# astaka-pe/SeMIGCN

Hardware: AMD Instinct MI355X
Metric: GCN train iters/sec + edges-aggregated/sec, 1M-vert mesh (higher is better)
Workload: dtype bf16 storage / f32 accumulate; 1 GPU; SGCN train iteration (13 ChebConv K=3 + BN + LeakyReLU, fwd+loss+bwd, Adam every 5th) on a closed torus mesh 1000x1000: V=1000000 E=6000000 directed, grid vertex order, bf16 features; V=1000000, E=6000000, vertex_order=grid

## Files before the change

include/semigcn.h:

```cpp
#ifndef SEMIGCN_H
#define SEMIGCN_H

#include <stdint.h>

#ifdef __cplusplus
extern "C" {
#endif

#if defined(__GNUC__)
#define SG_API __attribute__((visibility("default")))
#else
#define SG_API
#endif

#define SG_ABI_VERSION 1

enum sg_status {
  SG_OK = 0,
  SG_ERR_INVALID = -1,
  SG_ERR_HIP = -2,
  SG_ERR_UNSUPPORTED = -3,
  SG_ERR_NO_DEVICE = -4
};

enum sg_dtype {
  SG_F32 = 0,
  SG_BF16 = 1
};

typedef struct sg_graph sg_graph;
typedef struct sg_pool sg_pool;

SG_API const char* sg_last_error(void);
SG_API int sg_abi_version(void);
SG_API int sg_device_count(void);

SG_API int sg_graph_create(const int64_t* edge_index, int64_t E, int64_t V, void* stream, sg_graph** out);

SG_API int sg_graph_create_rect(const int64_t* dst, const int64_t* src, int64_t n, int64_t V_dst,
                         int64_t V_src, const float* dis_src, void* stream, sg_graph** out);

SG_API int sg_graph_create_rows(const int64_t* dst_pos, const int64_t* src, int64_t n, int64_t n_rows, int64_t V_src,
                                const int32_t* row_id, const float* dis_rows, const float* dis_src, void* stream,
                                sg_graph** out);

SG_API int sg_graph_destroy(sg_graph* g);

typedef struct sg_graph_info {
  int64_t V_dst, V_src;
  int64_t nnz;
  int32_t symmetric;
  int32_t max_degree;
} sg_graph_info;
SG_API int sg_graph_query(const sg_graph* g, sg_graph_info* info);
SG_API int sg_graph_is_reordered(const sg_graph* g);
SG_API int sg_graph_export(const sg_graph* g, int32_t* rowptr, int32_t* colidx, float* dis, void* stream);

SG_API int sg_graph_prepare(const sg_graph* g, int64_t C, int dtype, void* stream);
SG_API int sg_spmm(const sg_graph* g, int transpose, const void* X, int64_t ldx, const void* X0,
            int64_t ldx0, const void* X1, int64_t ldx1, void* Y, int64_t ldy, int64_t C, int dtype,
            float alpha, float beta, float gamma, void* stream);

SG_API int sg_pool_create(const int64_t* fine, const int64_t* coarse, int64_t n, int64_t n_fine,
                   int64_t n_coarse, void* stream, sg_pool** out);
SG_API int sg_pool_destroy(sg_pool* p);
SG_API int sg_pool_mean(const sg_pool* p, const void* X, int64_t ldx, void* Y, int64_t ldy, int64_t C,
                 int dtype, void* stream);
SG_API int sg_pool_mean_bwd(const sg_pool* p, const void* dY, int64_t lddy, void* dX, int64_t lddx,
                     int64_t C, int dtype, void* stream);
SG_API int sg_unpool(const sg_pool* p, const void* X, int64_t ldx, void* Y, int64_t ldy, int64_t C,
              int dtype, void* stream);
SG_API int sg_unpool_bwd(const sg_pool* p, const void* dY, int64_t lddy, void* dX, int64_t lddx,
                  int64_t C, int dtype, void* stream);

SG_API int sg_gather_rows(const int32_t* rows, int64_t n, const void* X, int64_t ldx, void* Y,
                   int64_t ldy, int64_t C, int dtype, void* stream);

SG_API int sg_thin_supported(int64_t N, int64_t K);
SG_API int64_t sg_thin_tn_blocks(int64_t V);
SG_API int sg_thin_nt(const void* X, int64_t ldx, const float* W, int64_t ldw, const float* bias, void* Y, int64_t ldy,
                      int64_t V, int64_t N, int64_t K, int dtype, void* stream);
SG_API int sg_thin_tn(const void* A, int64_t lda, const void* B, int64_t ldb, int64_t V, int64_t N, int64_t K, int dtype,
                      float* workspace, float* out, int64_t ldo, void* stream);
SG_API int64_t sg_col_apply_blocks(int64_t V, int64_t C, int dtype);
SG_API int sg_bn_act_bwd_apply_colsum(const void* dA, int64_t ldda, const void* H, int64_t ldh, const float* scale,
                                      const float* shift, const float* mean, const float* invstd, const float* k,
                                      const float* c1, const float* c2, float slope, void* dH, int64_t lddh, int64_t V,
                                      int64_t C, int dtype, float* colsum_partial, float* colsum, void* stream);
SG_API int64_t sg_col_blocks(int64_t V);
SG_API int sg_col_moments(const void* X, int64_t ldx, int64_t V, int64_t C, int dtype, float* partial,
                          int64_t nb, void* stream);
SG_API int sg_bn_merge(const float* partial, int64_t nb, int64_t V, int64_t C, float* stats, void* stream);
SG_API int sg_bn_stats_finalize(const float* partial, int64_t nb, int64_t V, int64_t C, const float* gamma,
                                const float* beta, float* running_mean, float* running_var, float momentum, float eps,
                                float* out, int64_t* batches_tracked, void* stream);
SG_API int sg_bn_bwd_coeffs(const float* partial, int64_t nb, int64_t C, double N, const float* gamma,
                            const float* invstd, float* out, float* acc_dweight, float* acc_dbias, const float* count_dev,
                            void* stream);
SG_API int sg_bn_merge_tiles(const float* partial, int64_t n_tiles, int64_t rows_per_tile, int64_t V, int64_t C, float* stats,
                             float* count_out, void* stream);
SG_API int sg_bn_finalize_ranks(const float* all, int64_t world, int64_t C, const float* gamma, const float* beta,
                                float* running_mean, float* running_var, float momentum, float eps, float* out,
                                float* out_n, int64_t* batches_tracked, void* stream);
SG_API int sg_multi_add(int64_t n, const float* const* srcs, const int64_t* src_ld, const int64_t* rows, const int64_t* cols,
                        float* const* dsts, void* stream);
SG_API int sg_bn_finalize(const float* stats, double N, int64_t C, const float* gamma, const float* beta,
                          float* running_mean, float* running_var, float momentum, float eps, float* out,
                          void* stream);
SG_API int sg_scale_shift_act(const void* X, int64_t ldx, const float* scale, const float* shift, float slope,
                              void* Y, int64_t ldy, int64_t V, int64_t C, int dtype, void* stream);
SG_API int sg_bn_act_bwd_reduce(const void* dA, int64_t ldda, const void* H, int64_t ldh, const float* scale,
                                const float* shift, const float* mean, const float* invstd, float slope,
                                float* partial, int64_t nb, int64_t V, int64_t C, int dtype, void* stream);
SG_API int sg_bn_act_bwd_apply(const void* dA, int64_t ldda, const void* H, int64_t ldh, const float* scale,
// ... 209 lines not shown
```

semigcn_amd/capi.py:

```python
from __future__ import annotations

import ctypes
import functools
from array import array as _array
import os
from ctypes import POINTER, byref, c_char_p, c_float, c_int, c_int32, c_int64, c_void_p
from typing import Optional

import torch

_LIB_NAME = "libsemigcn_hip.so"
_LIB_PATH = os.path.join(os.path.dirname(os.path.abspath(__file__)), _LIB_NAME)

SG_F32, SG_BF16 = 0, 1
_DTYPES = {torch.float32: SG_F32, torch.bfloat16: SG_BF16}


class SemigcnLibraryError(RuntimeError):
    """libsemigcn_hip.so is absent / unloadable, or a call into it failed."""


class sg_graph_info(ctypes.Structure):
    _fields_ = [("V_dst", c_int64), ("V_src", c_int64), ("nnz", c_int64),
                ("symmetric", c_int32), ("max_degree", c_int32)]
# ... 1 lines not shown

class sg_block(ctypes.Structure):
    _fields_ = [("graph", c_void_p), ("pool", c_void_p),
                ("pool_mode", c_int32), ("dtype", c_int32), ("K", c_int32), ("order", c_int32), ("training", c_int32),
                ("refresh_weights", c_int32), ("need_dx", c_int32), ("reserved_", c_int32),
                ("V", c_int64), ("V_out", c_int64), ("Cin", c_int64), ("Cout", c_int64),
                ("momentum", c_float), ("eps", c_float), ("slope", c_float), ("reserved2_", c_float),
                ("W", c_void_p * 3), ("bias", c_void_p), ("gamma", c_void_p), ("beta", c_void_p),
                ("running_mean", c_void_p), ("running_var", c_void_p), ("batches_tracked", c_void_p),
                ("wpack", c_void_p), ("wpack_t", c_void_p), ("wpack32", c_void_p), ("wpack32_t", c_void_p), ("bias_k", c_void_p),
                ("wsplit", c_void_p), ("wsplit_t", c_void_p),
                ("X", c_void_p), ("ldx", c_int64), ("T", c_void_p), ("ldt", c_int64), ("H", c_void_p), ("stats", c_void_p),
                ("Y", c_void_p), ("ldy", c_int64),
                ("dY", c_void_p), ("lddy", c_int64), ("dX", c_void_p), ("lddx", c_int64), ("dW", c_void_p), ("dvec", c_void_p),
                ("acc_W", c_void_p * 3), ("acc_bias", c_void_p), ("acc_gamma", c_void_p), ("acc_beta", c_void_p),
                ("ws", c_void_p), ("ws_bytes", c_int64),
                ("phase", c_int32), ("world", c_int32), ("graph_wide", c_void_p), ("V_ext", c_int64), ("ldh", c_int64),
                ("local", c_void_p), ("stats_rows", c_void_p), ("gathered", c_void_p), ("gathered_ready", c_int32),
                ("reserved3_", c_int32), ("count", c_void_p), ("send_index", c_void_p), ("n_send", c_int64), ("send", c_void_p),
                ("recv", c_void_p), ("G", c_void_p)]


PHASE_CONV, PHASE_BN, PHASE_BWD_REDUCE, PHASE_BWD_A, PHASE_BWD_B = 1, 2, 4, 8, 16


class sg_part_step(ctypes.Structure):
    _fields_ = [("kind", c_int32), ("reserved_", c_int32), ("blocks", POINTER(sg_block)), ("n", c_int64),
                ("send", c_void_p), ("recv", c_void_p)]


STEP_BLOCKS, STEP_EXCHANGE, STEP_ALL_REDUCE, STEP_ALL_GATHER = 0, 1, 2, 3


class sg_trace_record(ctypes.Structure):
    _fields_ = [("kind", c_int32), ("dtype", c_int32), ("engine", c_int32), ("reserved_", c_int32),
                ("a", c_int64), ("b", c_int64), ("c", c_int64), ("ms", c_float), ("reserved2_", c_float)]


_SIGNATURES = {
    "sg_last_error": (c_char_p, []),
    "sg_abi_version": (c_int, []),
    "sg_device_count": (c_int, []),
    "sg_graph_create": (c_int, [c_void_p, c_int64, c_int64, c_void_p, POINTER(c_void_p)]),
    "sg_graph_create_rect": (c_int, [c_void_p, c_void_p, c_int64, c_int64, c_int64, c_void_p, c_void_p,
                                     POINTER(c_void_p)]),
    "sg_graph_create_rows": (c_int, [c_void_p, c_void_p, c_int64, c_int64, c_int64, c_void_p, c_void_p, c_void_p, c_void_p,
                                     POINTER(c_void_p)]),
    "sg_graph_destroy": (c_int, [c_void_p]),
    "sg_graph_query": (c_int, [c_void_p, POINTER(sg_graph_info)]),
    "sg_graph_is_reordered": (c_int, [c_void_p]),
    "sg_graph_export": (c_int, [c_void_p, c_void_p, c_void_p, c_void_p, c_void_p]),
    "sg_spmm": (c_int, [c_void_p, c_int, c_void_p, c_int64, c_void_p, c_int64, c_void_p, c_int64,
                        c_void_p, c_int64, c_int64, c_int, c_float, c_float, c_float, c_void_p]),
    "sg_graph_prepare": (c_int, [c_void_p, c_int64, c_int, c_void_p]),
    "sg_pool_create": (c_int, [c_void_p, c_void_p, c_int64, c_int64, c_int64, c_void_p, POINTER(c_void_p)]),
    "sg_pool_destroy": (c_int, [c_void_p]),
    "sg_pool_mean": (c_int, [c_void_p, c_void_p, c_int64, c_void_p, c_int64, c_int64, c_int, c_void_p]),
    "sg_pool_mean_bwd": (c_int, [c_void_p, c_void_p, c_int64, c_void_p, c_int64, c_int64, c_int, c_void_p]),
    "sg_unpool": (c_int, [c_void_p, c_void_p, c_int64, c_void_p, c_int64, c_int64, c_int, c_void_p]),
    "sg_unpool_bwd": (c_int, [c_void_p, c_void_p, c_int64, c_void_p, c_int64, c_int64, c_int, c_void_p]),
    "sg_tuning_set": (c_int, [c_int, c_int]),
    "sg_mesh_loss_blocks": (c_int64, [c_int64, c_int64]),
    "sg_mesh_loss_fwd": (c_int, [c_void_p] * 6 + [c_int64, c_int64, c_void_p, c_void_p]),
    "sg_mesh_loss_bwd": (c_int, [c_void_p] * 7 + [c_int64, c_int64, c_int64, c_void_p, c_void_p]),
    "sg_mesh_loss_bwd_det": (c_int, [c_void_p] * 7 + [c_int64, c_int64, c_int64, c_void_p, c_void_p, c_void_p, c_void_p]),
    "sg_col_blocks": (c_int64, [c_int64]),
    "sg_col_moments": (c_int, [c_void_p, c_int64, c_int64, c_int64, c_int, c_void_p, c_int64, c_void_p]),
    "sg_bn_merge": (c_int, [c_void_p, c_int64, c_int64, c_int64, c_void_p, c_void_p]),
    "sg_bn_stats_finalize": (c_int, [c_void_p, c_int64, c_int64, c_int64, c_void_p, c_void_p, c_void_p, c_void_p, c_float,
                                     c_float, c_void_p, c_void_p, c_void_p]),
    "sg_bn_stats_finalize_tiles": (c_int, [c_void_p, c_int64, c_int64, c_int64, c_int64, c_void_p, c_void_p, c_void_p,
                                           c_void_p, c_float, c_float, c_void_p, c_void_p, c_void_p]),
    "sg_gemm_nt_takes_big_tile": (c_int, [c_int64, c_int64, c_int64, c_int64, c_int64, c_int64]),
    "sg_gemm_tile_rows": (c_int64, [c_int64]),
    "sg_gemm_row_tiles": (c_int64, [c_int64, c_int64]),
    "sg_gemm_nt": (c_int, [c_void_p, c_int64, c_void_p, c_int64, c_void_p, c_void_p, c_int64, c_int64, c_int64, c_int64,
                           c_int, c_void_p, c_void_p]),
    "sg_gemm_nt_f32_supported": (c_int, [c_int64, c_int64, c_int64, c_int64, c_int64]),
    "sg_gemm_nt_f32_pays": (c_int, [c_int64, c_int64, c_int64]),
    "sg_gemm_nt_f32_variant": (c_int, [c_int64]),
    "sg_gemm_nt_f32_workspace": (c_int64, [c_int64, c_int64]),
    "sg_gemm_nt_f32": (c_int, [c_void_p, c_int64, c_void_p, c_int64, c_int64, c_void_p, c_void_p, c_int64, c_int64, c_int64,
                               c_int64, c_void_p, c_int64, c_void_p]),
    "sg_gemm_tn_f32_supported": (c_int, [c_int64, c_int64, c_int64, c_int64, c_int64]),
    "sg_gemm_tn_f32_workspace": (c_int64, [c_int64, c_int64, c_int64]),
    "sg_gemm_tn_f32": (c_int, [c_void_p, c_int64, c_void_p, c_int64, c_int64, c_int64, c_int64, c_void_p, c_int64, c_void_p,
                               c_int64, c_void_p]),
    "sg_gemm_tn_slabs": (c_int64, [c_int64, c_int64, c_int64]),
    "sg_gemm_tn_takes_big_tile": (c_int, [c_int64, c_int64, c_int64, c_int64, c_int64]),
    "sg_gemm_tn": (c_int, [c_void_p, c_int64, c_void_p, c_int64, c_int64, c_int64, c_int64, c_int, c_void_p, c_void_p, c_int64,
                           c_void_p]),
    "sg_thin_supported": (c_int, [c_int64, c_int64]),
    "sg_thin_tn_blocks": (c_int64, [c_int64]),
    "sg_thin_nt": (c_int, [c_void_p, c_int64, c_void_p, c_int64, c_void_p, c_void_p, c_int64, c_int64, c_int64, c_int64, c_int,
                           c_void_p]),
    "sg_thin_tn": (c_int, [c_void_p, c_int64, c_void_p, c_int64, c_int64, c_int64, c_int64, c_int, c_void_p, c_void_p, c_int64,
                           c_void_p]),
    "sg_bn_bwd_coeffs": (c_int, [c_void_p, c_int64, c_int64, ctypes.c_double, c_void_p, c_void_p, c_void_p, c_void_p,
                                 c_void_p, c_void_p, c_void_p]),
    "sg_bn_merge_tiles": (c_int, [c_void_p, c_int64, c_int64, c_int64, c_int64, c_void_p, c_void_p, c_void_p]),
    "sg_multi_add": (c_int, [c_int64, c_void_p, c_void_p, c_void_p, c_void_p, c_void_p, c_void_p]),
    "sg_input_bounds": (c_int, [c_void_p, c_int64, c_void_p, c_void_p, c_void_p, c_void_p, c_void_p]),
    "sg_input_prep_bwd_routed": (c_int, [c_void_p, c_int64, c_void_p, c_void_p, c_void_p, c_void_p, c_void_p, c_void_p, c_void_p,
                                         c_void_p, c_int64, c_int, c_void_p]),
    "sg_mesh_loss_finalize": (c_int, [c_void_p, c_int64, c_float, c_float, c_float, c_float, c_void_p, c_void_p]),
    "sg_bnf_blocks": (c_int64, [c_int64]),
# ... 203 lines not shown
        with _on_device(ei.device):
            _check(load().sg_graph_create(_ptr(ei), ei.shape[1], int(num_vertices), _stream(ei), byref(out)),
                   "sg_graph_create")
        return cls(out.value, ei.device)

    @classmethod
    def from_partition(cls, dst: torch.Tensor, src: torch.Tensor, n_owned: int, n_ext: int,
                       dis_ext: torch.Tensor) -> "GraphHandle":
        for t, n in ((dst, "dst"), (src, "src"), (dis_ext, "dis_ext")):
            _require_device(t, n)
        dst, src = dst.contiguous(), src.contiguous()
        dis_ext = dis_ext.contiguous().float()
        assert dst.dtype == torch.int64 and src.dtype == torch.int64 and dis_ext.numel() == n_ext
        out = c_void_p()
        with _on_device(dst.device):
            _check(load().sg_graph_create_rect(_ptr(dst), _ptr(src), dst.numel(), int(n_owned), int(n_ext),
                                               _ptr(dis_ext), _stream(dst), byref(out)),
                   "sg_graph_create_rect")
        return cls(out.value, dst.device)

    @classmethod
    def from_rows(cls, dst_pos: torch.Tensor, src: torch.Tensor, row_id: torch.Tensor, out_rows: int, n_ext: int,
                  dis_rows: torch.Tensor, dis_ext: torch.Tensor) -> "GraphHandle":
        for t, n in ((dst_pos, "dst_pos"), (src, "src"), (row_id, "row_id"), (dis_rows, "dis_rows"), (dis_ext, "dis_ext")):
            _require_device(t, n)
        dst_pos, src = dst_pos.contiguous().long(), src.contiguous().long()
        row_id = row_id.contiguous().to(torch.int32)
        dis_rows, dis_ext = dis_rows.contiguous().float(), dis_ext.contiguous().float()
        assert dis_rows.numel() == row_id.numel() and dis_ext.numel() == n_ext
        out = c_void_p()
        with _on_device(src.device):
            _check(load().sg_graph_create_rows(_ptr(dst_pos), _ptr(src), dst_pos.numel(), row_id.numel(), int(n_ext),
                                               _ptr(row_id), _ptr(dis_rows), _ptr(dis_ext), _stream(src), byref(out)),
                   "sg_graph_create_rows")
        h = cls(out.value, src.device)
        h.num_rows = int(out_rows)
        return h

    def arrays(self):
        rp = torch.empty(self.num_rows + 1, dtype=torch.int32, device=self.device)
        ci = torch.empty(self.nnz, dtype=torch.int32, device=self.device)
        ds = torch.empty(self.num_cols, dtype=torch.float32, device=self.device)
        with _on_device(self.device):
            _check(load().sg_graph_export(self._h, _ptr(rp), _ptr(ci), _ptr(ds), _stream(rp)), "sg_graph_export")
        return rp, ci, ds

    def prepare(self, C: int, dtype: torch.dtype) -> None:
        with _on_device(self.device):
            _check(load().sg_graph_prepare(self._h, int(C), _DTYPES[dtype], torch.cuda.current_stream(self.device).cuda_stream),
                   "sg_graph_prepare")

    def spmm(self, X: torch.Tensor, Y: torch.Tensor, *, alpha: float = 1.0, X0: Optional[torch.Tensor] = None,
             beta: float = 0.0, X1: Optional[torch.Tensor] = None, gamma: float = 0.0,
             transpose: bool = False) -> torch.Tensor:
        if _timer is None and X.is_cuda and X.dim() == 2 and Y.dim() == 2 and X.device.index == _current_device():
            dt = X.dtype
            code = _DTYPES.get(dt)
            C = X.shape[1]
            n_in, n_out = (self.num_rows, self.num_cols) if transpose else (self.num_cols, self.num_rows)
            sx, sy = X.stride(), Y.stride()
            ok = (code is not None and X.shape[0] == n_in and Y.dtype == dt and Y.device == X.device and Y.shape[0] == n_out
                  and Y.shape[1] == C and (C <= 1 or (sx[1] == 1 and sy[1] == 1)))
            p0 = l0 = p1 = l1 = 0
            if ok and X0 is not None:
                s0 = X0.stride()
                ok = (X0.dtype == dt and X0.device == X.device and X0.dim() == 2 and X0.shape[0] == n_out and X0.shape[1] == C
                      and (C <= 1 or s0[1] == 1))
                p0, l0 = X0.data_ptr(), (s0[0] if n_out > 1 else max(s0[0], C))
            if ok and X1 is not None:
                s1 = X1.stride()
                ok = (X1.dtype == dt and X1.device == X.device and X1.dim() == 2 and X1.shape[0] == n_out and X1.shape[1] == C
                      and (C <= 1 or s1[1] == 1))
                p1, l1 = X1.data_ptr(), (s1[0] if n_out > 1 else max(s1[0], C))
            if ok and _raw_stream is not None:
                rc = _lib.sg_spmm(self._h, 1 if transpose else 0, X.data_ptr(), sx[0] if n_in > 1 else max(sx[0], C),
                                  p0, l0, p1, l1, Y.data_ptr(), sy[0] if n_out > 1 else max(sy[0], C), C, code,
                                  alpha, beta, gamma, _raw_stream(X.device.index))
                if rc:
                    _check(rc, "sg_spmm")
                return Y
        return self._spmm_checked(X, Y, alpha, X0, beta, X1, gamma, transpose)

    def _spmm_checked(self, X, Y, alpha, X0, beta, X1, gamma, transpose) -> torch.Tensor:
        for t, n in ((X, "X"), (Y, "Y"), (X0, "X0"), (X1, "X1")):
            if t is not None:
                _require_device(t, n)
                if t.dtype != X.dtype:
                    raise SemigcnLibraryError(f"{n} dtype {t.dtype} != X dtype {X.dtype}")
        C = X.shape[1]
        n_in, n_out = (self.num_rows, self.num_cols) if transpose else (self.num_cols, self.num_rows)
        if X.shape[0] != n_in or Y.shape != (n_out, C):
            raise SemigcnLibraryError(f"spmm shape mismatch: X {tuple(X.shape)} Y {tuple(Y.shape)} "
                                      f"operator {n_out}x{n_in}")
        for t, n in ((X0, "X0"), (X1, "X1")):
            if t is not None and t.shape != (n_out, C):
                raise SemigcnLibraryError(f"{n} shape {tuple(t.shape)} != {(n_out, C)}")
        timer = _timer
        with _on_device(X.device):
            if timer is not None:
                ev0, ev1 = torch.cuda.Event(enable_timing=True), torch.cuda.Event(enable_timing=True)
                ev0.record()
            _check(load().sg_spmm(self._h, int(transpose), _ptr(X), _rows2d(X, "X"),
                                  _ptr(X0), 0 if X0 is None else _rows2d(X0, "X0"),
                                  _ptr(X1), 0 if X1 is None else _rows2d(X1, "X1"),
                                  _ptr(Y), _rows2d(Y, "Y"), C, dtype_code(X),
                                  float(alpha), float(beta), float(gamma), _stream(X)), "sg_spmm")
            if timer is not None:
                ev1.record()
                n_epi = int(X0 is not None) + int(X1 is not None)
                timer.records.append(((C, str(X.dtype).replace("torch.", ""), n_epi, self.rows_processed), ev0, ev1))
        return Y

    def dilate_bits(self, bits: torch.Tensor) -> torch.Tensor:
        _require_device(bits, "bits")
        if bits.dtype != torch.int64 or bits.dim() != 2 or bits.shape[0] != self.num_rows:
            raise SemigcnLibraryError(f"bits must be int64 [{self.num_rows}, W], got {bits.dtype} {tuple(bits.shape)}")
        bits = bits.contiguous()
        out = torch.empty_like(bits)
        with _on_device(bits.device):
            _check(load().sg_mask_dilate(self._h, _ptr(bits), _ptr(out), bits.shape[1], _stream(bits)),
                   "sg_mask_dilate")
        return out

    def close(self):
        if getattr(self, "_h", None) is not None and self._h.value:
            load().sg_graph_destroy(self._h)
            self._h = c_void_p(0)

    def __del__(self):
        try:
            self.close()
        except Exception:
            pass

# ... 127 lines not shown
    rpt = int(rows_per_tile) if rows_per_tile else (int(num_rows) + nb - 1) // nb
    base = out.data_ptr()
    with _on_device(partial.device):
        _check(load().sg_bn_merge_tiles(_ptr(partial), nb, rpt, int(num_rows), C, base, base + 8 * C, _stream(partial)),
               "sg_bn_merge_tiles")
    return out


def bn_finalize(stats: torch.Tensor, count: float, gamma: torch.Tensor, beta: torch.Tensor,
                running_mean: Optional[torch.Tensor], running_var: Optional[torch.Tensor], momentum: float,
                eps: float) -> torch.Tensor:
    C = stats.shape[1]
    out = torch.empty((4, C), dtype=torch.float32, device=stats.device)
    for t, n in ((running_mean, "running_mean"), (running_var, "running_var")):
        if t is not None:
            _f32vec(t, C, n)
    with _on_device(stats.device):
        _check(load().sg_bn_finalize(_ptr(stats), float(count), C, _ptr(_f32vec(gamma, C, "weight")),
                                     _ptr(_f32vec(beta, C, "bias")), _ptr(running_mean), _ptr(running_var),
                                     float(momentum), float(eps), _ptr(out), _stream(stats)), "sg_bn_finalize")
    return out


def bn_finalize_ranks(all_stats: torch.Tensor, gamma: torch.Tensor, beta: torch.Tensor,
                      running_mean: Optional[torch.Tensor], running_var: Optional[torch.Tensor], momentum: float,
                      eps: float, batches_tracked: Optional[torch.Tensor] = None):
    world, w = all_stats.shape
    C = (w - 1) // 2
    out = torch.empty((4, C), dtype=torch.float32, device=all_stats.device)
    n = torch.empty((1,), dtype=torch.float32, device=all_stats.device)
    with _on_device(all_stats.device):
        _check(load().sg_bn_finalize_ranks(_ptr(all_stats), world, C, _ptr(_f32vec(gamma, C, "weight")),
                                           _ptr(_f32vec(beta, C, "bias")), _ptr(running_mean), _ptr(running_var),
                                           float(momentum), float(eps), _ptr(out), _ptr(n),
                                           _counter(batches_tracked, all_stats), _stream(all_stats)),
               "sg_bn_finalize_ranks")
    return out, n


def bn_stats_finalize(partial: torch.Tensor, num_rows: int, gamma: torch.Tensor, beta: torch.Tensor,
                      running_mean: Optional[torch.Tensor], running_var: Optional[torch.Tensor], momentum: float,
                      eps: float, batches_tracked: Optional[torch.Tensor] = None) -> torch.Tensor:
    nb, _, C = partial.shape
    out = torch.empty((4, C), dtype=torch.float32, device=partial.device)
    for t, n in ((running_mean, "running_mean"), (running_var, "running_var")):
        if t is not None:
            _f32vec(t, C, n)
    with _on_device(partial.device):
        _check(load().sg_bn_stats_finalize(_ptr(partial), nb, int(num_rows), C, _ptr(_f32vec(gamma, C, "weight")),
                                           _ptr(_f32vec(beta, C, "bias")), _ptr(running_mean), _ptr(running_var),
                                           float(momentum), float(eps), _ptr(out), _counter(batches_tracked, partial),
                                           _stream(partial)), "sg_bn_stats_finalize")
    return out


def bn_stats_finalize_tiles(partial: torch.Tensor, rows_per_tile: int, num_rows: int, gamma: torch.Tensor,
                            beta: torch.Tensor, running_mean: Optional[torch.Tensor], running_var: Optional[torch.Tensor],
                            momentum: float, eps: float, batches_tracked: Optional[torch.Tensor] = None) -> torch.Tensor:
    nb, _, C = partial.shape
    out = torch.empty((4, C), dtype=torch.float32, device=partial.device)
    for t, n in ((running_mean, "running_mean"), (running_var, "running_var")):
        if t is not None:
            _f32vec(t, C, n)
    with _on_device(partial.device):
        _check(load().sg_bn_stats_finalize_tiles(_ptr(partial), nb, int(rows_per_tile), int(num_rows), C,
                                                 _ptr(_f32vec(gamma, C, "weight")), _ptr(_f32vec(beta, C, "bias")),
                                                 _ptr(running_mean), _ptr(running_var), float(momentum), float(eps),
                                                 _ptr(out), _counter(batches_tracked, partial), _stream(partial)),
               "sg_bn_stats_finalize_tiles")
    return out


def gemm_tile_rows(N: int) -> int:
    return _sizes("sg_gemm_tile_rows", int(N))


def gemm_nt_supported(A: torch.Tensor, B: torch.Tensor, ldc: int) -> bool:
    if A.dtype != torch.bfloat16 or B.dtype != torch.bfloat16 or not A.is_cuda or A.dim() != 2 or B.dim() != 2:
        return False
    if A.shape[1] != B.shape[1] or A.stride(1) != 1 or B.stride(1) != 1 or A.shape[0] == 0:
        return False
    K, N = A.shape[1], B.shape[0]
    return (K % 8 == 0 and N % 8 == 0 and A.stride(0) % 8 == 0 and B.stride(0) % 8 == 0 and ldc % 8 == 0
            and A.data_ptr() % 16 == 0 and B.data_ptr() % 16 == 0)


def gemm_nt_takes_big_tile(M: int, N: int, K: int, lda: int, ldb: int, ldc: int) -> bool:
    return bool(_sizes("sg_gemm_nt_takes_big_tile", int(M), int(N), int(K), int(lda), int(ldb), int(ldc)))


def gemm_nt(A: torch.Tensor, B: torch.Tensor, bias: Optional[torch.Tensor] = None, out: Optional[torch.Tensor] = None,
            moments: bool = False):
    _require_device(A, "A")
    _require_device(B, "B")
    M, K = A.shape
    N = B.shape[0]
    if out is None:
        out = torch.empty((M, N), dtype=torch.bfloat16, device=A.device)
    if out.shape != (M, N) or out.dtype != torch.bfloat16 or B.shape[1] != K:
        raise SemigcnLibraryError(f"gemm_nt shape mismatch: A {tuple(A.shape)} B {tuple(B.shape)} out {tuple(out.shape)}")
    if bias is not None:
        _f32vec(bias, N, "bias")
    mom = None
    if moments:
        mom = torch.empty((_sizes("sg_gemm_row_tiles", M, N), 2, N), dtype=torch.float32, device=A.device)
    with _on_device(A.device):
# ... 707 lines not shown
```

semigcn_amd/csrc/api.hip:

```cpp
#include <stdarg.h>

#include <new>

#include <mutex>

#include "sg_common.h"

namespace sg {

static thread_local std::string t_error;

void set_error(const char* fmt, ...) {
  char buf[1024];
  va_list ap;
  va_start(ap, fmt);
  vsnprintf(buf, sizeof(buf), fmt, ap);
  va_end(ap);
  t_error = buf;
}

namespace {

struct ScopedFree {
  void* p = nullptr;
  ~ScopedFree() { if (p) (void)hipFree(p); }
};

void destroy_graph(sg_graph* g) {
  if (!g) return;
  g->fwd.release();
  g->bwd.release();
  g->loc.release();
  if (g->row_id) (void)hipFree(g->row_id);
  if (g->dis_dst_loc) (void)hipFree(g->dis_dst_loc);
  if (g->dis_src && g->dis_src != g->dis_dst) (void)hipFree(g->dis_src);
  if (g->dis_dst) (void)hipFree(g->dis_dst);
  delete g;
}

void destroy_pool(sg_pool* p) {
  if (!p) return;
  p->by_coarse.release();
  p->by_fine.release();
  if (p->inv_count) (void)hipFree(p->inv_count);
  delete p;
}

int check_dense(const char* what, const void* X, int64_t ld, int64_t C) {
  SG_REQUIRE(X != nullptr, "%s: null pointer", what);
  SG_REQUIRE(ld >= C, "%s: row stride %lld < C %lld", what, (long long)ld, (long long)C);
  return SG_OK;
}

std::mutex g_rec_mu;
int build_pending_records(const Csr& c_, hipStream_t stream) {
  hipStreamCaptureStatus st = hipStreamCaptureStatusNone;
  if (hipStreamIsCapturing(stream, &st) != hipSuccess) (void)hipGetLastError();
  if (st != hipStreamCaptureStatusNone) return SG_OK;
  std::lock_guard<std::mutex> lock(g_rec_mu);
  Csr& c = const_cast<Csr&>(c_);
  if (!__atomic_load_n(&c.rec_pending, __ATOMIC_ACQUIRE)) return SG_OK;
  const int rc = build_ring_records(&c, c.pend_scale_src, c.pend_scale_dst, c.pend_row_id, stream);
  if (rc == SG_OK) __atomic_store_n(&c.rec_pending, false, __ATOMIC_RELEASE);
  return rc;
}

int run_csr(const Csr& c, const float* sd, const float* ss, const void* X, int64_t ldx,
            const void* X0, int64_t ldx0, const void* X1, int64_t ldx1, void* Y, int64_t ldy,
            int64_t C, int dtype, float alpha, float beta, float gamma, hipStream_t stream,
            const int32_t* row_id = nullptr) {
  SG_REQUIRE(C >= 0 && C <= INT32_MAX, "C out of range");
  if (c.n_rows == 0 || C == 0) return SG_OK;
  int rc;
  if ((rc = check_dense("X", X, ldx, C)) != SG_OK) return rc;
  if ((rc = check_dense("Y", Y, ldy, C)) != SG_OK) return rc;
  if (X0 && (rc = check_dense("X0", X0, ldx0, C)) != SG_OK) return rc;
  if (X1 && (rc = check_dense("X1", X1, ldx1, C)) != SG_OK) return rc;
  SG_REQUIRE(X != Y, "Y must not alias X");
  if (__atomic_load_n(&c.rec_pending, __ATOMIC_ACQUIRE) && (dtype == SG_BF16 || (dtype == SG_F32 && ring_f32_enabled())) && (C == 128 || C == 256) &&
      (rc = build_pending_records(c, stream)) != SG_OK)
    return rc;
  SpmmArgs a;
  a.rowptr = c.rowptr;
  a.idx = c.idx;
  if (c.tile_rows == kTileRows) {
    a.tile_uptr = c.tile_uptr;
    a.tile_uniq = c.tile_uniq;
    a.tile_eloc = c.tile_eloc;
  }
  if (ss != nullptr && ss == c.packed_scale) {
    a.idx_w = c.idx_w;
    a.tile_uniq_w = c.tile_uniq_w;
    if (c.lt_uptr && c.lt_uniq_w && c.idx_w) {
      a.lt_idx_w = c.idx_w;
      a.lt_uptr = c.lt_uptr;
      a.lt_eloc = c.lt_eloc;
      a.lt_uniq_w = c.lt_uniq_w;
    }
  }
  if (ss != nullptr && ss == c.packed_scale && c.lt_rec && sd == c.rec_scale_dst && row_id == c.rec_row_id) {
    a.lt_rec = c.lt_rec;
    a.lt_nrec = c.lt_nrec;
    a.lt_idx_w = c.idx_w;
  }
  a.row_id = row_id;
  a.scale_dst = sd;
  a.scale_src = ss;
  a.X = X; a.X0 = X0; a.X1 = X1; a.Y = Y;
  a.ldx = ldx; a.ldx0 = X0 ? ldx0 : 0; a.ldx1 = X1 ? ldx1 : 0; a.ldy = ldy;
  a.n_rows = (int32_t)c.n_rows;
  a.n_cols = c.n_cols;
  a.C = (int32_t)C;
  a.alpha = alpha; a.beta = beta; a.gamma = gamma;
  return launch_spmm(a, dtype, stream);
}

}
}

using namespace sg;

extern "C" {

SG_API const char* sg_last_error(void) { return t_error.c_str(); }

SG_API int sg_abi_version(void) { return SG_ABI_VERSION; }

SG_API int sg_device_count(void) {
  int n = 0;
  hipError_t e = hipGetDeviceCount(&n);
  if (e != hipSuccess) {
    set_error("hipGetDeviceCount failed: %s", hipGetErrorString(e));
    (void)hipGetLastError();
    return SG_ERR_NO_DEVICE;
  }
  return n;
}

SG_API int sg_graph_create(const int64_t* edge_index, int64_t E, int64_t V, void* stream_, sg_graph** out) {
  SG_REQUIRE(out != nullptr, "sg_graph_create: out is null");
  *out = nullptr;
  SG_REQUIRE(E >= 0 && V >= 0, "sg_graph_create: negative size");
  SG_REQUIRE(E == 0 || edge_index != nullptr, "sg_graph_create: edge_index is null");
  hipStream_t stream = (hipStream_t)stream_;
  sg_graph* g = new (std::nothrow) sg_graph();
  SG_REQUIRE(g != nullptr, "out of host memory");
  const int64_t* src = edge_index;
  const int64_t* dst = edge_index + E;
  ScopedFree kf, kb;
  int rc = SG_OK;
  do {
    if (E > 0) {
      if (hipMalloc(&kf.p, E * sizeof(uint64_t)) != hipSuccess ||
          hipMalloc(&kb.p, E * sizeof(uint64_t)) != hipSuccess) {
        set_error("hipMalloc of sort keys failed");
        rc = SG_ERR_HIP;
        break;
      }
    }
    if ((rc = build_csr(dst, src, E, V, V, true, stream, &g->fwd, (uint64_t*)kf.p)) != SG_OK) break;
    if ((rc = build_csr(src, dst, E, V, V, true, stream, &g->bwd, (uint64_t*)kb.p)) != SG_OK) break;
    if (hipMalloc((void**)&g->dis_dst, (V > 0 ? V : 1) * sizeof(float)) != hipSuccess) {
      set_error("hipMalloc of dis failed");
      rc = SG_ERR_HIP;
      break;
    }
    g->dis_src = g->dis_dst;
// ... 113 lines not shown
    if (rc == SG_OK) rc = pack_source_scale(&g->fwd, g->dis_src, stream);
    if (rc == SG_OK && ring_enabled()) g->fwd.defer_records(g->dis_src, g->dis_dst, g->row_id);
    if (rc == SG_OK && hipStreamSynchronize(stream) != hipSuccess) {
      set_error("stream sync failed in sg_graph_create_rows");
      rc = SG_ERR_HIP;
    }
  }
  if (rc != SG_OK) {
    destroy_graph(g);
    return rc;
  }
  g->symmetric = true;
  g->square = false;
  *out = g;
  return SG_OK;
}

SG_API int sg_graph_destroy(sg_graph* g) {
  destroy_graph(g);
  return SG_OK;
}

SG_API int sg_graph_query(const sg_graph* g, sg_graph_info* info) {
  SG_REQUIRE(g && info, "sg_graph_query: null argument");
  info->V_dst = g->fwd.n_rows;
  info->V_src = g->fwd.n_cols;
  info->nnz = g->fwd.nnz;
  info->symmetric = g->symmetric ? 1 : 0;
  info->max_degree = g->fwd.max_degree;
  return SG_OK;
}

SG_API int sg_graph_is_reordered(const sg_graph* g) {
  if (!g) {
    set_error("sg_graph_is_reordered: null graph");
    return SG_ERR_INVALID;
  }
  return (g->square && g->row_id) ? 1 : 0;
}

SG_API int sg_graph_export(const sg_graph* g, int32_t* rowptr, int32_t* colidx, float* dis, void* stream_) {
  SG_REQUIRE(g != nullptr, "sg_graph_export: null graph");
  hipStream_t stream = (hipStream_t)stream_;
  if (rowptr)
    SG_HIP_TRY(hipMemcpyAsync(rowptr, g->fwd.rowptr, (g->fwd.n_rows + 1) * sizeof(int32_t),
                              hipMemcpyDeviceToDevice, stream));
  if (colidx && g->fwd.nnz > 0)
    SG_HIP_TRY(hipMemcpyAsync(colidx, g->fwd.idx, g->fwd.nnz * sizeof(int32_t), hipMemcpyDeviceToDevice, stream));
  if (dis && g->fwd.n_cols > 0)
    SG_HIP_TRY(hipMemcpyAsync(dis, g->dis_src, g->fwd.n_cols * sizeof(float), hipMemcpyDeviceToDevice, stream));
  return SG_OK;
}

SG_API int sg_spmm(const sg_graph* g, int transpose, const void* X, int64_t ldx, const void* X0, int64_t ldx0,
            const void* X1, int64_t ldx1, void* Y, int64_t ldy, int64_t C, int dtype, float alpha,
            float beta, float gamma, void* stream) {
  SG_REQUIRE(g != nullptr, "sg_spmm: null graph");
  const bool t = transpose != 0;
  if (t && !g->square) {
    set_error("sg_spmm: transpose of a rectangular (partition) operator is not available; "
              "apply it owner-computes on exchanged gradient rows");
    return SG_ERR_UNSUPPORTED;
  }
  TraceScope trace(0, dtype, 0, C, (X0 ? 1 : 0) + (X1 ? 1 : 0), (t && !g->symmetric) ? g->bwd.n_rows : g->fwd.n_rows,
                   (hipStream_t)stream);
  if (g->square && g->symmetric && g->row_id && g->loc.rowptr)
    return run_csr(g->loc, g->dis_dst_loc, g->dis_src, X, ldx, X0, ldx0, X1, ldx1, Y, ldy, C, dtype, -alpha, beta, gamma,
                   (hipStream_t)stream, g->row_id);
  if (!g->square && g->row_id)
    return run_csr(g->fwd, g->dis_dst, g->dis_src, X, ldx, X0, ldx0, X1, ldx1, Y, ldy, C, dtype, -alpha, beta, gamma,
                   (hipStream_t)stream, g->row_id);
  const Csr& c = (t && !g->symmetric) ? g->bwd : g->fwd;
  return run_csr(c, g->dis_dst, g->dis_src, X, ldx, X0, ldx0, X1, ldx1, Y, ldy, C, dtype, -alpha,
                 beta, gamma, (hipStream_t)stream);
}

SG_API int sg_graph_prepare(const sg_graph* g, int64_t C, int dtype, void* stream) {
  SG_REQUIRE(g != nullptr, "sg_graph_prepare: null graph");
  if (!(C == 128 || C == 256) || !(dtype == SG_BF16 || (dtype == SG_F32 && ring_f32_enabled()))) return SG_OK;
  const Csr* all[3] = {&g->fwd, &g->bwd, &g->loc};
  for (const Csr* c : all) {
    if (!__atomic_load_n(&const_cast<Csr*>(c)->rec_pending, __ATOMIC_ACQUIRE)) continue;
    const int rc = build_pending_records(*c, (hipStream_t)stream);
    if (rc != SG_OK) return rc;
  }
  return SG_OK;
}

SG_API int sg_pool_create(const int64_t* fine, const int64_t* coarse, int64_t n, int64_t n_fine,
                   int64_t n_coarse, void* stream_, sg_pool** out) {
  SG_REQUIRE(out != nullptr, "sg_pool_create: out is null");
  *out = nullptr;
  SG_REQUIRE(n >= 0 && n_fine >= 0 && n_coarse >= 0, "sg_pool_create: negative size");
  hipStream_t stream = (hipStream_t)stream_;
  sg_pool* p = new (std::nothrow) sg_pool();
  SG_REQUIRE(p != nullptr, "out of host memory");
  int rc = build_csr(coarse, fine, n, n_coarse, n_fine, false, stream, &p->by_coarse, nullptr);
  if (rc == SG_OK) rc = build_csr(fine, coarse, n, n_fine, n_coarse, false, stream, &p->by_fine, nullptr);
  if (rc == SG_OK && hipMalloc((void**)&p->inv_count, (n_coarse > 0 ? n_coarse : 1) * sizeof(float)) != hipSuccess) {
    set_error("hipMalloc of inv_count failed");
    rc = SG_ERR_HIP;
  }
  if (rc == SG_OK) rc = degree_scale(p->by_coarse, false, p->inv_count, stream);
  if (rc == SG_OK && hipStreamSynchronize(stream) != hipSuccess) {
    set_error("stream sync failed in sg_pool_create");
    rc = SG_ERR_HIP;
  }
  if (rc != SG_OK) {
    destroy_pool(p);
    return rc;
  }
  *out = p;
  return SG_OK;
}

SG_API int sg_pool_destroy(sg_pool* p) {
  destroy_pool(p);
  return SG_OK;
}

SG_API int sg_pool_mean(const sg_pool* p, const void* X, int64_t ldx, void* Y, int64_t ldy, int64_t C, int dtype,
                 void* stream) {
  SG_REQUIRE(p != nullptr, "sg_pool_mean: null pool");
  TraceScope trace(3, dtype, 0, C, p->by_coarse.n_rows, p->by_coarse.n_cols, (hipStream_t)stream);
  return run_csr(p->by_coarse, p->inv_count, nullptr, X, ldx, nullptr, 0, nullptr, 0, Y, ldy, C, dtype,
                 1.f, 0.f, 0.f, (hipStream_t)stream);
}
// ... 109 lines not shown
                                const float* target_fn, const float* f_keep, const float* g, int64_t V, int64_t V_ext,
                                int64_t F, const sg_pool* incidence, float* corner_scratch, float* grad_pos, void* stream_) {
  SG_REQUIRE(V >= 0 && F >= 0 && V_ext >= V && g && (V_ext == 0 || grad_pos), "sg_mesh_loss_bwd_det: bad argument");
  SG_REQUIRE((V == 0 || (pos && target_pos && v_keep)) && (F == 0 || (pos && faces && target_fn && f_keep)),
             "sg_mesh_loss_bwd_det: null pointer");
  SG_REQUIRE(incidence && incidence->by_coarse.n_rows == V_ext && incidence->by_coarse.n_cols == 3 * F &&
                 (F == 0 || corner_scratch),
             "sg_mesh_loss_bwd_det: incidence must map the 3F face corners onto V_ext vertices");
  hipStream_t stream = (hipStream_t)stream_;
  int rc = launch_mesh_loss_bwd_corners(pos, faces, target_fn, f_keep, g, F, corner_scratch, stream);
  if (rc != SG_OK) return rc;
  if (V_ext == 0) return SG_OK;
  if (F == 0) {
    SG_HIP_TRY(hipMemsetAsync(grad_pos, 0, (size_t)V_ext * 3 * sizeof(float), stream));
  } else {
    rc = run_csr(incidence->by_coarse, nullptr, nullptr, corner_scratch, 3, nullptr, 0, nullptr, 0, grad_pos, 3, 3, SG_F32,
                 1.f, 0.f, 0.f, stream);
    if (rc != SG_OK) return rc;
  }
  return launch_mesh_loss_bwd_vertex_add(pos, target_pos, v_keep, g, V, grad_pos, stream);
}

SG_API int64_t sg_col_blocks(int64_t V) { return col_blocks(V); }

SG_API int sg_col_moments(const void* X, int64_t ldx, int64_t V, int64_t C, int dtype, float* partial, int64_t nb,
                          void* stream) {
  SG_REQUIRE(V >= 0 && C >= 0, "sg_col_moments: negative size");
  if (V == 0 || C == 0) return SG_OK;
  SG_REQUIRE(X && partial && ldx >= C, "sg_col_moments: bad argument");
  return launch_col_reduce(0, X, ldx, nullptr, 0, nullptr, nullptr, nullptr, nullptr, 0.f, partial, nb, V, C, dtype,
                           (hipStream_t)stream);
}

SG_API int sg_bn_merge(const float* partial, int64_t nb, int64_t V, int64_t C, float* stats, void* stream) {
  SG_REQUIRE(V > 0 && C >= 0 && partial && stats, "sg_bn_merge: bad argument");
  return launch_bn_merge(partial, nb, V, C, stats, (hipStream_t)stream);
}

SG_API int sg_bn_merge_tiles(const float* partial, int64_t n_tiles, int64_t rows_per_tile, int64_t V, int64_t C, float* stats,
                             float* count_out, void* stream) {
  SG_REQUIRE(V > 0 && C >= 0 && partial && stats, "sg_bn_merge_tiles: bad argument");
  return launch_bn_merge_tiles(partial, n_tiles, rows_per_tile, V, C, stats, count_out, (hipStream_t)stream);
}

SG_API int sg_bn_stats_finalize(const float* partial, int64_t nb, int64_t V, int64_t C, const float* gamma,
                                const float* beta, float* running_mean, float* running_var, float momentum, float eps,
                                float* out, int64_t* batches_tracked, void* stream) {
  SG_REQUIRE(V > 1 && C >= 0 && partial && gamma && beta && out, "sg_bn_stats_finalize: bad argument");
  SG_REQUIRE((running_mean == nullptr) == (running_var == nullptr),
             "sg_bn_stats_finalize: give both running buffers or none");
  return launch_bn_stats_finalize(partial, nb, V, C, gamma, beta, running_mean, running_var, momentum, eps, out,
                                  batches_tracked, (hipStream_t)stream);
}

SG_API int sg_bn_stats_finalize_tiles(const float* partial, int64_t n_tiles, int64_t rows_per_tile, int64_t V, int64_t C,
                                      const float* gamma, const float* beta, float* running_mean, float* running_var,
                                      float momentum, float eps, float* out, int64_t* batches_tracked, void* stream) {
  SG_REQUIRE(V > 1 && C >= 0 && partial && gamma && beta && out, "sg_bn_stats_finalize_tiles: bad argument");
  SG_REQUIRE((running_mean == nullptr) == (running_var == nullptr),
             "sg_bn_stats_finalize_tiles: give both running buffers or none");
  return launch_bn_stats_finalize_tiles(partial, n_tiles, rows_per_tile, V, C, gamma, beta, running_mean, running_var,
                                        momentum, eps, out, batches_tracked, (hipStream_t)stream);
}

SG_API int sg_gemm_nt_takes_big_tile(int64_t M, int64_t N, int64_t K, int64_t lda, int64_t ldb, int64_t ldc) {
  return gemm_nt_takes_big_tile(M, N, K, lda, ldb, ldc) ? 1 : 0;
}

SG_API int64_t sg_gemm_tile_rows(int64_t N) { return gemm_tile_rows(N); }

SG_API int64_t sg_gemm_row_tiles(int64_t M, int64_t N) {
  const int64_t r = gemm_tile_rows(N);
  return M <= 0 ? 0 : (M + r - 1) / r;
}

SG_API int sg_gemm_nt(const void* A, int64_t lda, const void* B, int64_t ldb, const float* bias, void* C, int64_t ldc,
                      int64_t M, int64_t N, int64_t K, int dtype, float* moments, void* stream) {
  SG_REQUIRE(M >= 0 && N >= 0 && K >= 0, "sg_gemm_nt: negative size");
  if (M == 0 || N == 0) return SG_OK;
  SG_REQUIRE(A && B && C && K > 0, "sg_gemm_nt: null operand or K = 0");
  SG_REQUIRE(lda >= K && ldb >= K && ldc >= N, "sg_gemm_nt: row stride shorter than the row");
  return launch_gemm_nt(A, lda, B, ldb, bias, C, ldc, M, N, K, dtype, moments, (hipStream_t)stream);
}

SG_API int64_t sg_gemm_tn_slabs(int64_t M, int64_t N, int64_t Kp) { return gemm_tn_slabs(M, N, Kp); }

SG_API int sg_gemm_tn_takes_big_tile(int64_t M, int64_t N, int64_t Kp, int64_t lda, int64_t ldb) {
  return gemm_tn_takes_big_tile(M, N, Kp, lda, ldb) ? 1 : 0;
}

SG_API int sg_gemm_tn(const void* A, int64_t lda, const void* B, int64_t ldb, int64_t M, int64_t N, int64_t Kp, int dtype,
                      float* workspace, float* out, int64_t ldo, void* stream) {
  SG_REQUIRE(M >= 0 && N >= 0 && Kp >= 0, "sg_gemm_tn: negative size");
  if (N == 0 || Kp == 0) return SG_OK;
  SG_REQUIRE(out != nullptr && ldo >= Kp, "sg_gemm_tn: bad output");
  if (M == 0) {
    SG_HIP_TRY(hipMemset2DAsync(out, ldo * sizeof(float), 0, Kp * sizeof(float), N, (hipStream_t)stream));
    return SG_OK;
  }
  SG_REQUIRE(A && B && workspace && lda >= N && ldb >= Kp, "sg_gemm_tn: null operand or short row stride");
  return launch_gemm_tn(A, lda, B, ldb, M, N, Kp, dtype, workspace, out, ldo, (hipStream_t)stream);
}

SG_API int sg_gemm_nt_f32_supported(int64_t M, int64_t N, int64_t K, int64_t lda, int64_t ldc) {
  return (gemm_nt_f32s_supported(M, N, K, lda, ldc) || (M >= 0 && mid_shape(N, K) && lda % 4 == 0 && ldc % 4 == 0)) ? 1 : 0;
}
// ... 253 lines not shown
```

semigcn_amd/csrc/block.hip:

```cpp
#include <math.h>

#include "sg_common.h"

namespace sg {
namespace {

bool g_block_planes = true;

inline int64_t esize(int dtype) { return dtype == SG_F32 ? 4 : 2; }
inline int64_t align_up(int64_t v) { return (v + 255) & ~(int64_t)255; }

struct Carver {
  char* base;
  int64_t cap, at = 0;
  bool overflow = false;
  Carver(void* b, int64_t c) : base((char*)b), cap(c) {}
  void* take(int64_t bytes) {
    const int64_t off = at;
    at += align_up(bytes > 0 ? bytes : 1);
    if (!base) return nullptr;
    if (at > cap) {
      overflow = true;
      return nullptr;
    }
// ... 88 lines not shown
  } else if (b.pool_mode == 2) {
    SG_REQUIRE(b.pool && b.pool->by_fine.n_cols == b.V && b.pool->by_fine.n_rows == b.V_out,
               "sg_block: MeshUnpool handle does not map %lld coarse rows onto %lld fine rows", (long long)b.V, (long long)b.V_out);
  } else {
    set_error("sg_block: pool_mode %d", b.pool_mode);
    return SG_ERR_INVALID;
  }
  if (b.training) SG_REQUIRE(b.V_out > 1, "sg_block: BatchNorm in training mode needs more than one row");
  s->V = b.V; s->Vo = b.V_out; s->Ci = b.Cin; s->Co = b.Cout; s->K = b.K;
  s->KCi = b.K * b.Cin; s->KCo = b.K * b.Cout; s->e = esize(b.dtype);
  if (col_apply_blocks(b.V_out, b.Cout, b.dtype) == 0) {
    set_error("sg_block: Cout = %lld is not served (whole 16-byte vectors, at most 256 of them per row)", (long long)b.Cout);
    return SG_ERR_UNSUPPORTED;
  }
  if (b.order == 0) {
    s->thin = thin_shape(s->Co, s->KCi);
    s->blas_fwd = !s->thin && !dense_nt_own(b.dtype, s->V, s->Co, s->KCi, s->KCi, s->KCi, s->Co);
    s->blas_dx = !s->thin && !dense_nt_own(b.dtype, s->V, s->KCi, s->Co, s->Co, s->Co, s->KCi);
    s->blas_dw = !s->thin && !dense_tn_own(b.dtype, s->V, s->Co, s->KCi, s->Co, s->KCi);
    s->tn_floats = dense_tn_workspace(b.dtype, s->V, s->Co, s->KCi);
  } else {
    s->thin = false;
    s->blas_fwd = !dense_nt_own(b.dtype, s->V, s->KCo, s->Ci, s->Ci, s->Ci, s->KCo);
    s->blas_dx = !dense_nt_own(b.dtype, s->V, s->Ci, s->KCo, s->KCo, s->KCo, s->Ci);
    s->blas_dw = !dense_tn_own(b.dtype, s->V, s->KCo, s->Ci, s->KCo, s->Ci) || thin_shape(s->KCo, s->Ci);
    s->tn_floats = thin_shape(s->KCo, s->Ci) ? 0 : dense_tn_workspace(b.dtype, s->V, s->KCo, s->Ci);
    if (thin_shape(s->KCo, s->Ci)) {
      set_error("sg_block: order 1 with a %lld x %lld weight stack is not served", (long long)s->KCo, (long long)s->Ci);
      return SG_ERR_UNSUPPORTED;
    }
  }
  {
    const int64_t C = b.order == 0 ? s->Ci : s->Co;
    int lg = 0;
    while ((1 << lg) < C) ++lg;
    bool ok = b.dtype == SG_BF16 && b.K > 1 && (1 << lg) == C && C >= 8 && C <= 64 && g_block_planes;
    if (ok && b.order == 0)
      ok = dense_planes_ok_nt(b.dtype, s->V, s->Co, s->KCi) && dense_planes_ok_nt(b.dtype, s->V, s->KCi, s->Co) &&
           dense_planes_ok_tn(b.dtype, s->V, s->Co, s->KCi);
    else if (ok)
      ok = dense_planes_ok_nt(b.dtype, s->V, s->KCo, s->Ci) && dense_planes_ok_nt(b.dtype, s->V, s->Ci, s->KCo) &&
           dense_planes_ok_tn(b.dtype, s->V, s->KCo, s->Ci);
    s->planes_ok = ok;
    s->pl = Planes{};
    if (ok) {
      s->pl.log2 = lg;
      s->pl.stride = s->V * C;
    }
  }
  s->nb = col_blocks(s->Vo);
  const int64_t R = gemm_tile_rows(s->Co);
  const int64_t tiles = (s->V + R - 1) / R;
  s->mom_floats = (tiles > s->nb ? tiles : s->nb) * 2 * s->Co;
  return SG_OK;
}

struct FwdWs {
  float* moments;
  void* Z;
  void* Hc;
  void* blas;
};
void carve_fwd(const sg_block& b, const Shape& s, Carver& c, FwdWs* w) {
  w->moments = (float*)c.take(s.mom_floats * 4);
  w->Z = b.order == 1 ? c.take(s.V * s.KCo * s.e) : nullptr;
  w->Hc = b.pool_mode ? c.take(s.V * s.Co * s.e) : nullptr;
  w->blas = s.blas_fwd ? c.take((int64_t)kBlasWorkspace) : nullptr;
}

struct BwdWs {
  float* part;
  float* colsum;
  void* dHp;
  void* dHc;
  void* G;
  float* tn;
  void* blas;
};
void carve_bwd(const sg_block& b, const Shape& s, Carver& c, BwdWs* w) {
  w->part = (float*)c.take(s.nb * 2 * s.Co * 4);
  w->colsum = (float*)c.take(col_apply_blocks(s.Vo, s.Co, b.dtype) * s.Co * 4);
  const bool sep = b.order == 0 || b.pool_mode != 0;
  w->dHp = sep ? c.take(s.Vo * s.Co * s.e) : nullptr;
  w->dHc = (b.order == 0 && b.pool_mode) ? c.take(s.V * s.Co * s.e) : nullptr;
  w->G = c.take(s.V * (b.order == 0 ? s.KCi : s.KCo) * s.e);
  w->tn = (float*)c.take(s.tn_floats * 4);
  w->blas = (s.blas_dx || s.blas_dw) ? c.take((int64_t)kBlasWorkspace) : nullptr;
}

int spmm(const sg_block& b, bool transpose, const void* X, int64_t ldx, const void* X0, int64_t ldx0, const void* X1,
         int64_t ldx1, void* Y, int64_t ldy, int64_t C, float alpha, float beta, float gamma, hipStream_t s) {
  return sg_spmm(b.graph, transpose ? 1 : 0, X, ldx, X0, ldx0, X1, ldx1, Y, ldy, C, b.dtype, alpha, beta, gamma, (void*)s);
}

inline char* col(void* base, int64_t cols, int64_t e) { return (char*)base + cols * e; }

inline bool split_image_shape(int64_t N, int64_t K) { return N >= 64 && N % 4 == 0 && K >= 64 && K % 32 == 0; }
inline const void* split_image(const sg_block& b, bool transposed, int64_t N, int64_t K) {
  return (b.dtype == SG_F32 && split_image_shape(N, K)) ? (transposed ? b.wsplit_t : b.wsplit) : nullptr;
}

int pack(const sg_block& b, hipStream_t stream) {
  SG_REQUIRE(b.wpack != nullptr, "sg_block: wpack is null");
  PackArgs a;
  for (int k = 0; k < 3; ++k) a.W[k] = k < b.K ? b.W[k] : nullptr;
  for (int k = 0; k < b.K; ++k) SG_REQUIRE(b.W[k] != nullptr, "sg_block: W[%d] is null", k);
  a.bias = b.bias;
  a.wpack = b.wpack; a.wpack_t = b.wpack_t; a.wpack32 = b.wpack32; a.wpack32_t = b.wpack32_t;
  a.bias_k = (b.order == 1 && b.bias) ? b.bias_k : nullptr;
  a.K = b.K; a.Cin = (int)b.Cin; a.Cout = (int)b.Cout; a.order = b.order; a.dtype = b.dtype;
  const int64_t n = (int64_t)b.K * b.Cin * b.Cout;
  pack_weights<<<(int)((n + 255) / 256), 256, 0, stream>>>(a);
  SG_HIP_TRY(hipGetLastError());
  if (b.dtype == SG_F32 && (b.wsplit || b.wsplit_t)) {
    const int64_t na = b.order == 0 ? b.Cout : (int64_t)b.K * b.Cout, ka = b.order == 0 ? (int64_t)b.K * b.Cin : b.Cin;
    const float* const w32 = (const float*)b.wpack;
    if (b.wsplit && split_image_shape(na, ka)) {
      int rc = launch_pack_split(w32, ka, 1, b.V, na, ka, b.wsplit, stream);
      if (rc != SG_OK) return rc;
    }
    if (b.wsplit_t && split_image_shape(ka, na)) {
      int rc = launch_pack_split(w32, 1, ka, b.V, ka, na, b.wsplit_t, stream);
      if (rc != SG_OK) return rc;
    }
  }
  return SG_OK;
}

int t_layout(const sg_block& b, const Shape& s, const char* who, Planes* pt) {
  *pt = Planes{};
  SG_REQUIRE(b.T != nullptr, "%s: order 0 needs the [V, K*Cin] buffer T", who);
  if (b.K > 1 && b.ldt == s.Ci) {
    SG_REQUIRE(s.planes_ok, "%s: T given as K planes (ldt == Cin) for a shape that does not take them (sg_block_planar)", who);
    *pt = s.pl;
    return SG_OK;
  }
  SG_REQUIRE(b.ldt >= s.KCi, "%s: row stride of T shorter than K*Cin", who);
  return SG_OK;
}

int forward(const sg_block& b, hipStream_t stream) {
  Shape s;
  int rc = shape_of(b, &s);
  if (rc != SG_OK) return rc;
  SG_REQUIRE(b.X && b.H && b.Y && b.stats && b.gamma && b.beta && b.wpack, "sg_block_forward: null pointer");
  SG_REQUIRE(b.ldy >= s.Co && b.ldx >= s.Ci, "sg_block_forward: row stride shorter than the row");
  SG_REQUIRE((b.running_mean == nullptr) == (b.running_var == nullptr), "sg_block_forward: give both running buffers or none");
  SG_REQUIRE(b.training || b.running_mean, "sg_block_forward: eval mode needs the running statistics");
  if (s.thin) SG_REQUIRE(b.wpack32 && b.wpack32_t, "sg_block_forward: a tiny weight matrix needs wpack32 / wpack32_t");
  if (b.order == 1 && b.bias) SG_REQUIRE(b.bias_k != nullptr, "sg_block_forward: order 1 with a bias needs bias_k");
  Carver c(b.ws, b.ws_bytes);
  FwdWs w;
  carve_fwd(b, s, c, &w);
  SG_REQUIRE(b.ws != nullptr && !c.overflow, "sg_block_forward: scratch too small (%lld bytes given, %lld needed)",
             (long long)b.ws_bytes, (long long)c.at);
  if (b.refresh_weights && (rc = pack(b, stream)) != SG_OK) return rc;

  void* const Hc = b.pool_mode ? w.Hc : b.H;
  bool tile_moments = false;
  if (b.order == 0) {
    Planes pt;
    if ((rc = t_layout(b, s, "sg_block_forward", &pt)) != SG_OK) return rc;
    auto t = [&](int k) { return pt.on() ? col(b.T, k * pt.stride, s.e) : col(b.T, k * s.Ci, s.e); };
    if (b.X != b.T && (rc = copy_rows(b.X, b.ldx, b.T, b.ldt, s.V, s.Ci, b.dtype, stream)) != SG_OK) return rc;
    for (int k = 1; k < b.K; ++k) {
      rc = spmm(b, false, t(k - 1), b.ldt, k >= 2 ? t(k - 2) : nullptr, b.ldt, nullptr, 0, t(k), b.ldt, s.Ci, k == 1 ? 1.f : 2.f,
                -1.f, 0.f, stream);
      if (rc != SG_OK) return rc;
    }
    const bool want = b.training && b.pool_mode == 0;
    rc = dense_nt(b.T, b.ldt, b.wpack, b.wpack32, s.KCi, b.bias, Hc, s.Co, s.V, s.Co, s.KCi, b.dtype, want ? w.moments : nullptr,
                  &tile_moments, w.blas, kBlasWorkspace, stream, pt, Planes{}, split_image(b, false, s.Co, s.KCi), b.V);
    if (rc != SG_OK) return rc;
  } else {
    const Planes pz = s.planes_ok ? s.pl : Planes{};
    const int64_t ldz = pz.on() ? s.Co : s.KCo;
    rc = dense_nt(b.X, b.ldx, b.wpack, nullptr, s.Ci, b.bias ? b.bias_k : nullptr, w.Z, ldz, s.V, s.KCo, s.Ci, b.dtype, nullptr,
                  nullptr, w.blas, kBlasWorkspace, stream, Planes{}, pz, split_image(b, false, s.KCo, s.Ci), b.V);
    if (rc != SG_OK) return rc;
    auto z = [&](int k) { return pz.on() ? col(w.Z, k * pz.stride, s.e) : col(w.Z, k * s.Co, s.e); };
    for (int k = b.K - 2; k >= 1; --k) {
      rc = spmm(b, false, z(k + 1), ldz, z(k), ldz, k + 2 <= b.K - 1 ? z(k + 2) : nullptr, ldz, z(k), ldz, s.Co, 2.f, 1.f, -1.f,
                stream);
      if (rc != SG_OK) return rc;
    }
    rc = spmm(b, false, z(1), ldz, z(0), ldz, b.K >= 3 ? z(2) : nullptr, ldz, Hc, s.Co, s.Co, 1.f, 1.f, -1.f, stream);
    if (rc != SG_OK) return rc;
  }
  if (b.pool_mode == 1) rc = sg_pool_mean(b.pool, Hc, s.Co, b.H, s.Co, s.Co, b.dtype, (void*)stream);
  else if (b.pool_mode == 2) rc = sg_unpool(b.pool, Hc, s.Co, b.H, s.Co, s.Co, b.dtype, (void*)stream);
  if (rc != SG_OK) return rc;

  if (b.training) {
    if (tile_moments) {
      const int64_t R = gemm_tile_rows(s.Co);
      rc = launch_bn_stats_finalize_tiles(w.moments, (s.V + R - 1) / R, R, s.Vo, s.Co, b.gamma, b.beta, b.running_mean,
                                          b.running_var, b.momentum, b.eps, b.stats, b.batches_tracked, stream);
    } else {
      rc = launch_col_reduce(0, b.H, s.Co, nullptr, 0, nullptr, nullptr, nullptr, nullptr, 0.f, w.moments, s.nb, s.Vo, s.Co,
                             b.dtype, stream);
      if (rc != SG_OK) return rc;
      rc = launch_bn_stats_finalize(w.moments, s.nb, s.Vo, s.Co, b.gamma, b.beta, b.running_mean, b.running_var, b.momentum,
                                    b.eps, b.stats, b.batches_tracked, stream);
    }
    if (rc != SG_OK) return rc;
  } else {
    bn_eval_coeffs<<<(int)((s.Co + 127) / 128), 128, 0, stream>>>(b.running_mean, b.running_var, b.gamma, b.beta, b.eps,
                                                                 (int)s.Co, b.stats);
    SG_HIP_TRY(hipGetLastError());
  }
  return launch_col_apply(0, b.H, s.Co, nullptr, 0, b.stats + 2 * s.Co, b.stats + 3 * s.Co, nullptr, nullptr, nullptr, nullptr,
                          nullptr, b.slope, b.Y, b.ldy, s.Vo, s.Co, b.dtype, stream);
}

int backward(const sg_block& b, hipStream_t stream) {
  Shape s;
  int rc = shape_of(b, &s);
  if (rc != SG_OK) return rc;
  SG_REQUIRE(b.dY && b.H && b.stats && b.gamma && b.dW && b.dvec && b.wpack, "sg_block_backward: null pointer");
  SG_REQUIRE(b.lddy >= s.Co, "sg_block_backward: row stride of dY shorter than the row");
  SG_REQUIRE(!b.need_dx || (b.dX && b.lddx >= s.Ci), "sg_block_backward: need_dx without dX");
  SG_REQUIRE((b.acc_gamma == nullptr) == (b.acc_beta == nullptr), "sg_block_backward: give both BatchNorm accumulators or none");
  const bool sink_w = b.acc_W[0] != nullptr;
  for (int k = 0; k < b.K; ++k)
    SG_REQUIRE((b.acc_W[k] != nullptr) == sink_w, "sg_block_backward: give all K weight accumulators or none");
  if (s.thin) SG_REQUIRE(b.wpack32 && b.wpack32_t, "sg_block_backward: a tiny weight matrix needs wpack32 / wpack32_t");
  Carver c(b.ws, b.ws_bytes);
  BwdWs w;
  carve_bwd(b, s, c, &w);
  SG_REQUIRE(b.ws != nullptr && !c.overflow, "sg_block_backward: scratch too small (%lld bytes given, %lld needed)",
             (long long)b.ws_bytes, (long long)c.at);
  const float *mean = b.stats, *invstd = b.stats + s.Co, *scale = b.stats + 2 * s.Co, *shift = b.stats + 3 * s.Co;
  float* const co = b.dvec;
  float* const db = b.dvec + 5 * s.Co;

  rc = launch_col_reduce(1, b.dY, b.lddy, b.H, s.Co, scale, shift, mean, invstd, b.slope, w.part, s.nb, s.Vo, s.Co, b.dtype, stream);
  if (rc != SG_OK) return rc;
  rc = launch_bn_bwd_coeffs(w.part, s.nb, s.Co, b.training ? (double)s.Vo : (double)INFINITY, b.gamma, invstd, co, b.acc_gamma,
                            b.acc_beta, nullptr, stream);
  if (rc != SG_OK) return rc;
  const Planes pg = (b.order == 1 && s.planes_ok) ? s.pl : Planes{};
  const int64_t ldg = pg.on() ? s.Co : s.KCo;
  void* dHp = w.dHp;
  int64_t lddh = s.Co;
  if (b.order == 1 && b.pool_mode == 0) {
    dHp = w.G;
    lddh = ldg;
  }
  rc = launch_col_apply(1, b.dY, b.lddy, b.H, s.Co, scale, shift, mean, invstd, co + 4 * s.Co, co + 2 * s.Co, co + 3 * s.Co, b.slope,
                        dHp, lddh, s.Vo, s.Co, b.dtype, stream, w.colsum);
// ... 443 lines not shown
```

semigcn_amd/csrc/bn_act.hip:

```cpp
#include <type_traits>

#include "sg_common.h"

namespace sg {
namespace {

constexpr int kBlock = 256;

typedef float f32x4 __attribute__((ext_vector_type(4)));
typedef uint32_t u32x4 __attribute__((ext_vector_type(4)));

template <int DT> struct Io;
template <> struct Io<SG_F32> {
  static constexpr int VEC = 4;
  using raw = f32x4;
  using elem = float;
  static __device__ __forceinline__ void unpack(const raw& v, float* f) { f[0] = v.x; f[1] = v.y; f[2] = v.z; f[3] = v.w; }
  static __device__ __forceinline__ raw pack(const float* f) { return raw{f[0], f[1], f[2], f[3]}; }
  static __device__ __forceinline__ float load1(const elem* p) { return *p; }
  static __device__ __forceinline__ void store1(elem* p, float v) { *p = v; }
};
template <> struct Io<SG_BF16> {
  static constexpr int VEC = 8;
  using raw = u32x4;
// ... 322 lines not shown
      int64_t rows = V - b * rpb;
      rows = rows > rpb ? rpb : rows;
      if (rows <= 0) break;
      const double nbk = (double)rows, mb = partial[(b * 2 + 0) * C + c], qb = partial[(b * 2 + 1) * C + c];
      const double tot = n + nbk, delta = mb - mean;
      mean += delta * (nbk / tot);
      m2 += qb + delta * delta * (n * nbk / tot);
      n = tot;
    }
  }
#pragma unroll
  for (int off = 32; off > 0; off >>= 1) {
    const double n2 = __shfl_down(n, off, 64), mean2 = __shfl_down(mean, off, 64), m22 = __shfl_down(m2, off, 64);
    const double tot = n + n2;
    if (tot > 0.0) {
      const double delta = mean2 - mean;
      mean += delta * (n2 / tot);
      m2 += m22 + delta * delta * (n * n2 / tot);
      n = tot;
    }
  }
  if (c < C && lane == 0) {
    stats[c] = (float)mean;
    stats[C + c] = (float)m2;
    if (count_out && c == 0) count_out[0] = (float)V;
  }
}

__global__ void bn_finalize(const float* __restrict__ stats, double N, int C, const float* __restrict__ gamma,
                            const float* __restrict__ beta, float* running_mean, float* running_var,
                            float momentum, float eps, float* __restrict__ out ) {
  const int c = blockIdx.x * blockDim.x + threadIdx.x;
  if (c >= C) return;
  const float mean = stats[c];
  const double m2 = stats[C + c];
  const float var = (float)(m2 / N);
  const float invstd = rsqrtf(var + eps);
  const float scale = gamma[c] * invstd;
  out[c] = mean;
  out[C + c] = invstd;
  out[2 * C + c] = scale;
  out[3 * C + c] = beta[c] - mean * scale;
  if (running_mean) {
    running_mean[c] = (1.f - momentum) * running_mean[c] + momentum * mean;
    running_var[c] = (1.f - momentum) * running_var[c] + momentum * (float)(m2 / (N - 1.0));
  }
}

__global__ __launch_bounds__(256) void bn_stats_finalize(const float* __restrict__ partial, int64_t nb, int64_t V, int C,
                                                         int rpb, const float* __restrict__ gamma,
                                                         const float* __restrict__ beta, float* running_mean,
                                                         float* running_var, float momentum, float eps,
                                                         float* __restrict__ out ,
                                                         long long* batches_tracked) {
  __shared__ double s_n[4], s_mean[4], s_m2[4];
  const int lane = threadIdx.x & 63, wave = threadIdx.x >> 6;
  const int c = blockIdx.x;
  double n = 0.0, mean = 0.0, m2 = 0.0;
  for (int64_t b = threadIdx.x; b < nb; b += 256) {
    int64_t rows = V - b * rpb;
    rows = rows > rpb ? rpb : rows;
    if (rows <= 0) break;
    const double nbk = (double)rows, mb = partial[(b * 2 + 0) * C + c], qb = partial[(b * 2 + 1) * C + c];
    const double tot = n + nbk, delta = mb - mean;
    mean += delta * (nbk / tot);
    m2 += qb + delta * delta * (n * nbk / tot);
    n = tot;
  }
#pragma unroll
  for (int off = 32; off > 0; off >>= 1) {
    const double n2 = __shfl_down(n, off, 64), mean2 = __shfl_down(mean, off, 64), m22 = __shfl_down(m2, off, 64);
    const double tot = n + n2;
    if (tot > 0.0) {
      const double delta = mean2 - mean;
      mean += delta * (n2 / tot);
      m2 += m22 + delta * delta * (n * n2 / tot);
      n = tot;
    }
  }
  if (lane == 0) { s_n[wave] = n; s_mean[wave] = mean; s_m2[wave] = m2; }
  __syncthreads();
  if (threadIdx.x == 0) {
    for (int w = 1; w < 4; ++w) {
      const double n2 = s_n[w], tot = n + n2;
      if (tot > 0.0 && n2 > 0.0) {
        const double delta = s_mean[w] - mean;
        mean += delta * (n2 / tot);
        m2 += s_m2[w] + delta * delta * (n * n2 / tot);
        n = tot;
      }
    }
    const float meanf = (float)mean;
    const double m2d = (double)(float)m2;
    const double N = (double)V;
    const float invstd = rsqrtf((float)(m2d / N) + eps);
    const float scale = gamma[c] * invstd;
    out[c] = meanf;
    out[C + c] = invstd;
    out[2 * C + c] = scale;
    out[3 * C + c] = beta[c] - meanf * scale;
    if (running_mean) {
      running_mean[c] = (1.f - momentum) * running_mean[c] + momentum * meanf;
      running_var[c] = (1.f - momentum) * running_var[c] + momentum * (float)(m2d / (N - 1.0));
    }
    if (batches_tracked && c == 0) *batches_tracked += 1;
  }
}

__global__ __launch_bounds__(256) void bn_bwd_coeffs(const float* __restrict__ partial, int64_t nb, int C, double N,
                                                     const float* __restrict__ gamma, const float* __restrict__ invstd,
                                                     float* __restrict__ out , float* acc_dweight,
                                                     float* acc_dbias, const float* __restrict__ count_dev) {
  __shared__ double s_w0[4], s_w1[4];
  if (count_dev) N = (double)count_dev[0];
  const int c = blockIdx.x;
  double s0 = 0.0, s1 = 0.0;
// ... 80 lines not shown
  return t;
}

}

int64_t col_blocks(int64_t V) {
  int64_t nb = (V + 127) / 128;
  if (nb < 1) nb = 1;
  if (nb > 2048) nb = 2048;
  return nb;
}

int launch_bn_merge(const float* partial, int64_t nb, int64_t V, int64_t C, float* stats, hipStream_t stream) {
  if (C == 0) return SG_OK;
  SG_REQUIRE(nb == col_blocks(V), "partial buffer must have sg_col_blocks(V) blocks");
  const int rpb = (int)((V + nb - 1) / nb);
  bn_merge<<<(int)((C + 3) / 4), 256, 0, stream>>>(partial, nb, V, (int)C, rpb, stats, nullptr);
  SG_HIP_TRY(hipGetLastError());
  return SG_OK;
}

int launch_bn_merge_tiles(const float* partial, int64_t nb, int64_t rpb, int64_t V, int64_t C, float* stats,
                          float* count_out, hipStream_t stream) {
  if (C == 0) return SG_OK;
  SG_REQUIRE(rpb > 0 && rpb <= INT32_MAX && nb >= (V + rpb - 1) / rpb, "partial buffer must have >= ceil(V / rows_per_tile) tiles");
  bn_merge<<<(int)((C + 3) / 4), 256, 0, stream>>>(partial, nb, V, (int)C, (int)rpb, stats, count_out);
  SG_HIP_TRY(hipGetLastError());
  return SG_OK;
}

int launch_bn_stats_finalize(const float* partial, int64_t nb, int64_t V, int64_t C, const float* gamma,
                             const float* beta, float* running_mean, float* running_var, float momentum, float eps,
                             float* out, int64_t* batches_tracked, hipStream_t stream) {
  if (C == 0) return SG_OK;
  SG_REQUIRE(nb == col_blocks(V), "partial buffer must have sg_col_blocks(V) blocks");
  const int rpb = (int)((V + nb - 1) / nb);
  bn_stats_finalize<<<(int)C, 256, 0, stream>>>(partial, nb, V, (int)C, rpb, gamma, beta, running_mean, running_var,
                                                momentum, eps, out, (long long*)batches_tracked);
  SG_HIP_TRY(hipGetLastError());
  return SG_OK;
}

int launch_bn_stats_finalize_tiles(const float* partial, int64_t nb, int64_t rpb, int64_t V, int64_t C, const float* gamma,
                                   const float* beta, float* running_mean, float* running_var, float momentum, float eps,
                                   float* out, int64_t* batches_tracked, hipStream_t stream) {
  if (C == 0) return SG_OK;
  SG_REQUIRE(rpb > 0 && rpb <= INT32_MAX && nb == (V + rpb - 1) / rpb, "partial buffer must have ceil(V / rows_per_tile) tiles");
  bn_stats_finalize<<<(int)C, 256, 0, stream>>>(partial, nb, V, (int)C, (int)rpb, gamma, beta, running_mean, running_var,
                                                momentum, eps, out, (long long*)batches_tracked);
  SG_HIP_TRY(hipGetLastError());
  return SG_OK;
}

int launch_multi_add(int n, const float* const* srcs, const int64_t* src_ld, const int64_t* rows, const int64_t* cols,
                     float* const* dsts, hipStream_t stream) {
  MultiAddArgs a{};
  a.n = n;
  int64_t at = 0;
  for (int s = 0; s < n; ++s) {
    a.src[s] = srcs[s];
    a.dst[s] = dsts[s];
    a.ld[s] = src_ld[s];
    a.cols[s] = (int)(cols[s] > 0 ? cols[s] : 1);
    a.start[s] = at;
    at += rows[s] * cols[s];
  }
  a.start[n] = at;
  if (at == 0) return SG_OK;
  int64_t blocks = (at + 1023) / 1024;
  if (blocks > 1024) blocks = 1024;
  multi_add<<<(int)blocks, 256, 0, stream>>>(a);
  SG_HIP_TRY(hipGetLastError());
  return SG_OK;
}

int launch_bn_bwd_coeffs(const float* partial, int64_t nb, int64_t C, double N, const float* gamma,
                         const float* invstd, float* out, float* acc_dweight, float* acc_dbias, const float* count_dev,
                         hipStream_t stream) {
  if (C == 0) return SG_OK;
  bn_bwd_coeffs<<<(int)C, 256, 0, stream>>>(partial, nb, (int)C, N, gamma, invstd, out, acc_dweight, acc_dbias,
                                                        count_dev);
  SG_HIP_TRY(hipGetLastError());
  return SG_OK;
}

int launch_bn_finalize_ranks(const float* all, int64_t world, int64_t C, const float* gamma, const float* beta,
                             float* running_mean, float* running_var, float momentum, float eps, float* out,
                             float* out_n, int64_t* batches_tracked, hipStream_t stream) {
  if (C == 0) return SG_OK;
  bn_finalize_ranks<<<(int)((C + 127) / 128), 128, 0, stream>>>(all, (int)world, (int)C, gamma, beta, running_mean,
                                                               running_var, momentum, eps, out, out_n,
                                                               (long long*)batches_tracked);
  SG_HIP_TRY(hipGetLastError());
  return SG_OK;
}

int launch_bn_finalize(const float* stats, double N, int64_t C, const float* gamma, const float* beta,
                       float* running_mean, float* running_var, float momentum, float eps, float* out,
                       hipStream_t stream) {
  if (C == 0) return SG_OK;
  bn_finalize<<<(int)((C + 127) / 128), 128, 0, stream>>>(stats, N, (int)C, gamma, beta, running_mean, running_var,
                                                         momentum, eps, out);
  SG_HIP_TRY(hipGetLastError());
  return SG_OK;
}

int launch_col_reduce(int mode, const void* A, int64_t lda, const void* H, int64_t ldh, const float* scale,
                      const float* shift, const float* mean, const float* invstd, float slope, float* out,
                      int64_t nblk, int64_t V, int64_t C, int dtype, hipStream_t stream) {
  if (V == 0 || C == 0) return SG_OK;
  SG_REQUIRE(nblk == col_blocks(V), "partial buffer must have sg_col_blocks(V) = %lld blocks", (long long)col_blocks(V));
  const int rpb = (int)((V + nblk - 1) / nblk);
  auto run = [&](auto dt_tag) -> int {
    constexpr int DT = decltype(dt_tag)::value;
    constexpr int VEC = Io<DT>::VEC;
    const bool vec = C % VEC == 0 && lda % VEC == 0 && a16(A) && (mode == 0 || (ldh % VEC == 0 && a16(H)));
    const int ncol = vec ? (int)(C / VEC) : (int)C;
    const int tpr = threads_per_row(ncol);
#define SG_LAUNCH(MODE, VW) col_reduce<DT, MODE, VW><<<(int)nblk, kBlock, 0, stream>>>(A, lda, H, ldh, scale, shift, mean, invstd, slope, out, V, (int)C, rpb, tpr)
    if (mode == 0) { if (vec) SG_LAUNCH(0, VEC); else SG_LAUNCH(0, 1); }
    else { if (vec) SG_LAUNCH(1, VEC); else SG_LAUNCH(1, 1); }
#undef SG_LAUNCH
    SG_HIP_TRY(hipGetLastError());
    return SG_OK;
  };
  if (dtype == SG_F32) return run(std::integral_constant<int, SG_F32>{});
  if (dtype == SG_BF16) return run(std::integral_constant<int, SG_BF16>{});
  set_error("unsupported dtype %d", dtype);
  return SG_ERR_UNSUPPORTED;
}

int64_t col_apply_blocks(int64_t V, int64_t C, int dtype) {
  const int VEC = dtype == SG_F32 ? 4 : 8;
  if (C % VEC || C / VEC > kBlock || V <= 0) return 0;
  const int ncol = (int)(C / VEC);
  int lg = 0;
  while ((1 << lg) < ncol) ++lg;
  const int groups = kBlock >> lg;
  int64_t nbr = (V + (int64_t)groups * 4 - 1) / ((int64_t)groups * 4);
  if (nbr > 256 * 16) nbr = 256 * 16;
  return nbr < 1 ? 1 : nbr;
}

int launch_colsum_finalize(const float* partial, int64_t nb, int64_t C, float* out, hipStream_t stream, float* acc) {
  if (C == 0) return SG_OK;
  colsum_finalize<<<(int)C, 256, 0, stream>>>(partial, nb, (int)C, out, acc);
  SG_HIP_TRY(hipGetLastError());
  return SG_OK;
}

int g_bn_rows_contiguous = 0;
int set_bn_rows_tuning(int value) {
  g_bn_rows_contiguous = value;
  return SG_OK;
}

int launch_col_apply(int mode, const void* A, int64_t lda, const void* H, int64_t ldh, const float* scale,
                     const float* shift, const float* mean, const float* invstd, const float* kk, const float* c1,
                     const float* c2, float slope, void* Y, int64_t ldy, int64_t V, int64_t C, int dtype,
                     hipStream_t stream, float* colsum) {
  if (V == 0 || C == 0) return SG_OK;
  auto run = [&](auto dt_tag) -> int {
    constexpr int DT = decltype(dt_tag)::value;
// ... 41 lines not shown
```

semigcn_amd/csrc/sg_common.h:

```cpp
#pragma once
#include <hip/hip_runtime.h>
#include <stdint.h>
#include <stdio.h>
#include <atomic>
#include <string>

#include "semigcn.h"

namespace sg {

void set_error(const char* fmt, ...);

#define SG_HIP_TRY(expr)                                                              \
  do {                                                                                \
    hipError_t e__ = (expr);                                                          \
    if (e__ != hipSuccess) {                                                          \
      sg::set_error("%s failed: %s (%s:%d)", #expr, hipGetErrorString(e__), __FILE__, \
                    __LINE__);                                                        \
      return SG_ERR_HIP;                                                              \
    }                                                                                 \
  } while (0)

#define SG_REQUIRE(cond, ...)      \
  do {                             \
// ... 3 lines not shown
    }                              \
  } while (0)

struct Csr {
  int64_t n_rows = 0, n_cols = 0, nnz = 0;
  int32_t* rowptr = nullptr;
  int32_t* idx = nullptr;
  int32_t max_degree = 0;
  int32_t tile_rows = 0;
  int32_t* tile_uptr = nullptr;
  int32_t* tile_uniq = nullptr;
  uint8_t* tile_eloc = nullptr;
  int2* idx_w = nullptr;
  int2* tile_uniq_w = nullptr;
  int32_t* lt_uptr = nullptr;
  int32_t* lt_uniq = nullptr;
  uint8_t* lt_eloc = nullptr;
  int2* lt_uniq_w = nullptr;
  uint8_t* lt_rec = nullptr;
  int32_t lt_nrec = 0;
  const float* rec_scale_dst = nullptr;
  const int32_t* rec_row_id = nullptr;
  bool rec_pending = false;
  const float* pend_scale_src = nullptr;
  const float* pend_scale_dst = nullptr;
  const int32_t* pend_row_id = nullptr;
  void defer_records(const float* ss, const float* sd, const int32_t* rid) {
    rec_pending = true;
    pend_scale_src = ss;
    pend_scale_dst = sd;
    pend_row_id = rid;
  }
  const float* packed_scale = nullptr;
  void release();
};

constexpr int kTileRows = 4;
constexpr int kTileSlots = 32;
constexpr int kTileEdges = 128;
constexpr int kLdsRows = 16;
constexpr int kLdsSlots = 48;
constexpr int kLdsEdges = 256;
constexpr int kRingSlots = 56;
constexpr int kRecSrc = 0;
constexpr int kRecSlot = kRecSrc + 4 * kRingSlots;
constexpr int kRecDeg = kRecSlot + 16 * kLdsRows;
constexpr int kRecNu = kRecDeg + kLdsRows;
constexpr int kRecE0 = kRecNu + 4;
constexpr int kRecR0 = kRecE0 + 4;
constexpr int kRecNrows = kRecR0 + 4;
constexpr int kRecSd = kRecNrows + 4;
constexpr int kRecRow = kRecSd + 4 * kLdsRows;
constexpr int kRecW = kRecRow + 4 * kLdsRows;
constexpr int kRecBytes = 896;
static_assert(kRecW + 4 * kRingSlots <= kRecBytes && kRecSd % 16 == 0, "tile record layout");
int build_tiles(Csr* c, hipStream_t stream);
int pack_source_scale(Csr* c, const float* scale, hipStream_t stream);
struct GradSink {
  float* dst[3] = {nullptr, nullptr, nullptr};
  int mode = 0, Cin = 0, Cout = 0;
  const float* cs_partial = nullptr;
  int64_t cs_nb = 0;
  int cs_C = 0;
  float* cs_out = nullptr;
  float* cs_acc = nullptr;
};
#ifdef __HIPCC__
__device__ inline void colsum_ride(const GradSink& s, int c) {
  __shared__ double s_ride[4];
  double v = 0.0;
  if (threadIdx.x < 256)
    for (int64_t b = threadIdx.x; b < s.cs_nb; b += 256) v += s.cs_partial[b * s.cs_C + c];
#pragma unroll
  for (int off = 32; off > 0; off >>= 1) v += __shfl_down(v, off, 64);
  if (threadIdx.x < 256 && (threadIdx.x & 63) == 0) s_ride[threadIdx.x >> 6] = v;
  __syncthreads();
  if (threadIdx.x == 0) {
    const double t = (s_ride[0] + s_ride[1]) + (s_ride[2] + s_ride[3]);
    s.cs_out[c] = (float)t;
    if (s.cs_acc) s.cs_acc[c] += (float)t;
  }
}
#endif
__device__ __forceinline__ float* sink_ptr(const GradSink& s, int64_t n, int64_t kk) {
  if (s.mode == 1) {
    const int64_t k = kk / s.Cin;
    return s.dst[k] + n * s.Cin + (kk - k * s.Cin);
  }
  const int64_t k = n / s.Cout;
  return s.dst[k] + (n - k * s.Cout) * s.Cin + kk;
}
struct Planes {
  int log2 = 31;
  int64_t stride = 0;
  bool on() const { return log2 != 31; }
};
__host__ __device__ __forceinline__ int64_t plane_off(int c, int log2, int64_t stride) {
  return (int64_t)(c >> log2) * stride + (c & (int)((1u << log2) - 1u));
}
bool thin_shape(int64_t N, int64_t K);
int64_t thin_tn_blocks(int64_t V);
int launch_thin_nt(const void* X, int64_t ldx, const float* W, int64_t ldw, const float* bias, void* Y, int64_t ldy, int64_t V,
                   int64_t N, int64_t K, int dtype, hipStream_t stream);
int launch_thin_tn(const void* A, int64_t lda, const void* B, int64_t ldb, int64_t V, int64_t N, int64_t K, int dtype,
                   float* workspace, float* out, int64_t ldo, hipStream_t stream, const GradSink* sink = nullptr);
int build_ring_records(Csr* c, const float* scale_src, const float* scale_dst, const int32_t* row_id, hipStream_t stream);
bool ring_enabled();
bool ring_f32_enabled();

int build_csr(const int64_t* dst, const int64_t* src, int64_t n, int64_t n_rows, int64_t n_cols,
              bool drop_self, hipStream_t stream, Csr* out, uint64_t* keys_out);

int degree_scale(const Csr& c, bool inv_sqrt, float* out, hipStream_t stream);
int locality_order(const Csr& c, int mode, hipStream_t stream, int32_t** order_out);
int permute_rows(const Csr& base, const int32_t* order, hipStream_t stream, Csr* out);
int gather_floats(const float* src, const int32_t* order, int64_t n, float* out, hipStream_t stream);
int graph_reorder_mode();
int set_graph_reorder_mode(int v);
int keys_equal(const uint64_t* a, const uint64_t* b, int64_t n, hipStream_t stream, int* equal);

struct SpmmArgs {
  const int32_t* rowptr;
  const int32_t* idx;
  const int32_t* tile_uptr = nullptr;
  const int32_t* tile_uniq = nullptr;
  const uint8_t* tile_eloc = nullptr;
  const int2* idx_w = nullptr;
  const int2* tile_uniq_w = nullptr;
  const int32_t* lt_uptr = nullptr;
  const uint8_t* lt_eloc = nullptr;
  const int2* lt_uniq_w = nullptr;
  const int2* lt_idx_w = nullptr;
  const uint8_t* lt_rec = nullptr;
  int32_t lt_nrec = 0;
  const int32_t* row_id = nullptr;
  const float* scale_dst;
  const float* scale_src;
  const void* X;
  const void* X0;
  const void* X1;
  void* Y;
  int64_t ldx, ldx0, ldx1, ldy;
  int32_t n_rows;
  int64_t n_cols = 0;
  int32_t C;
  float alpha, beta, gamma;
};

int launch_spmm(const SpmmArgs& a, int dtype, hipStream_t stream);
int set_tuning(int knob, int value);
bool tiles_enabled();
bool lds_tiles_enabled();
int launch_gather_rows(const int32_t* rows, int64_t n, const void* X, int64_t ldx, void* Y,
                       int64_t ldy, int64_t C, int dtype, hipStream_t stream);

int64_t col_blocks(int64_t V);
int launch_col_reduce(int mode, const void* A, int64_t lda, const void* H, int64_t ldh, const float* scale,
                      const float* shift, const float* mean, const float* invstd, float slope, float* out,
                      int64_t nblk, int64_t V, int64_t C, int dtype, hipStream_t stream);
int launch_bn_merge(const float* partial, int64_t nb, int64_t V, int64_t C, float* stats, hipStream_t stream);
int launch_bn_stats_finalize(const float* partial, int64_t nb, int64_t V, int64_t C, const float* gamma,
                             const float* beta, float* running_mean, float* running_var, float momentum, float eps,
                             float* out, int64_t* batches_tracked, hipStream_t stream);
int launch_bn_bwd_coeffs(const float* partial, int64_t nb, int64_t C, double N, const float* gamma,
                         const float* invstd, float* out, float* acc_dweight, float* acc_dbias, const float* count_dev,
                         hipStream_t stream);
int launch_bn_merge_tiles(const float* partial, int64_t nb, int64_t rpb, int64_t V, int64_t C, float* stats,
                          float* count_out, hipStream_t stream);
int launch_bn_finalize_ranks(const float* all, int64_t world, int64_t C, const float* gamma, const float* beta,
                             float* running_mean, float* running_var, float momentum, float eps, float* out,
                             float* out_n, int64_t* batches_tracked, hipStream_t stream);
int launch_bn_finalize(const float* stats, double N, int64_t C, const float* gamma, const float* beta,
                       float* running_mean, float* running_var, float momentum, float eps, float* out,
                       hipStream_t stream);
int launch_col_apply(int mode, const void* A, int64_t lda, const void* H, int64_t ldh, const float* scale,
                     const float* shift, const float* mean, const float* invstd, const float* kk, const float* c1,
                     const float* c2, float slope, void* Y, int64_t ldy, int64_t V, int64_t C, int dtype,
                     hipStream_t stream, float* colsum = nullptr);
int64_t col_apply_blocks(int64_t V, int64_t C, int dtype);
int launch_colsum_finalize(const float* partial, int64_t nb, int64_t C, float* out, hipStream_t stream, float* acc = nullptr);

int launch_bn_stats_finalize_tiles(const float* partial, int64_t nb, int64_t rpb, int64_t V, int64_t C, const float* gamma,
                                   const float* beta, float* running_mean, float* running_var, float momentum, float eps,
                                   float* out, int64_t* batches_tracked, hipStream_t stream);
constexpr int kMultiAddMax = 8;
int launch_multi_add(int n, const float* const* srcs, const int64_t* src_ld, const int64_t* rows, const int64_t* cols,
                     float* const* dsts, hipStream_t stream);

int64_t input_prep_blocks(int64_t V);
int launch_input_prep(const float* z1, const float* dm, const int64_t* order, const float* lo, const float* hi, void* X,
                      int64_t ldx, int64_t V, int dtype, hipStream_t stream);
int launch_input_prep_bwd(const void* gX, int64_t ldg, const float* z1, const float* dm, const int64_t* rank, const float* lo,
                          const float* hi, float* dz1, float* partial, float* d_lo, float* d_hi, int64_t V, int dtype,
                          hipStream_t stream);

int launch_input_bounds(const float* z1, int64_t V, float* pv, int64_t* pi, float* bounds, int64_t* arg, hipStream_t stream);
int launch_bounds_route(const float* d_lo, const float* d_hi, const int64_t* arg, float* dz1, hipStream_t stream);
int launch_mesh_loss_finalize(const float* partial, int64_t nb, float n_v, float n_f, float w_pos, float k1, float* out,
                              hipStream_t stream);

int gemm_tile_rows(int64_t N);
int set_gemm_tuning(int value);
int launch_gemm_nt(const void* A, int64_t lda, const void* B, int64_t ldb, const float* bias, void* C, int64_t ldc,
                   int64_t M, int64_t N, int64_t K, int dtype, float* moments, hipStream_t stream, Planes pa = {}, Planes pc = {});

bool gemm_nt_takes_big_tile(int64_t M, int64_t N, int64_t K, int64_t lda, int64_t ldb, int64_t ldc);
bool gemm_nt_256_supported(int64_t M, int64_t N, int64_t K, int64_t lda, int64_t ldb, int64_t ldc);
int launch_gemm_nt_256(const void* A, int64_t lda, const void* B, int64_t ldb, const float* bias, void* C, int64_t ldc,
                       int64_t M, int64_t N, int64_t K, hipStream_t stream);
bool gemm_tn_256_supported(int64_t M, int64_t N, int64_t Kp, int64_t lda, int64_t ldb);
int gemm_tn_256_slabs(int64_t M, int64_t N, int64_t Kp);
int launch_gemm_tn_256(const void* A, int64_t lda, const void* B, int64_t ldb, int64_t M, int64_t N, int64_t Kp,
                       float* workspace, hipStream_t stream);
bool gemm_tn_takes_big_tile(int64_t M, int64_t N, int64_t Kp, int64_t lda, int64_t ldb);
int64_t gemm_tn_slabs(int64_t M, int64_t N, int64_t Kp);
int launch_gemm_tn(const void* A, int64_t lda, const void* B, int64_t ldb, int64_t M, int64_t N, int64_t Kp, int dtype,
// ... 114 lines not shown
```

semigcn_amd/csrc/spmm.hip:

```cpp
#include "sg_common.h"

namespace sg {
namespace {

constexpr int kBlock = 256;
constexpr int kWaves = kBlock / 64;
constexpr int kChMax = 64;
constexpr int kCap = 512;

struct bf16_tag {};
typedef float f32x4 __attribute__((ext_vector_type(4)));
typedef uint32_t u32x4 __attribute__((ext_vector_type(4)));

enum : int { kFlagXcdMap = 1, kFlagNoTiles = 2, kFlagNoPackedScale = 4, kFlagBlockBarrier = 8, kFlagWideAddr = 16, kFlagNoExact = 32,
             kFlagStreamEpilogue = 64, kFlagLdsTiles = 128, kFlagNoQuad = 256, kFlagThreadRows = 512, kFlagNoRing = 2048, kFlagRingDirectStores = 4096,
             kFlagNoRingF32 = 8192 };

__device__ __forceinline__ void wave_sync(int flags) {
  if (flags & kFlagBlockBarrier) {
    __syncthreads();
  } else {
    __builtin_amdgcn_fence(__ATOMIC_RELEASE, "wavefront");
    __builtin_amdgcn_wave_barrier();
    __builtin_amdgcn_fence(__ATOMIC_ACQUIRE, "wavefront");
// ... 635 lines not shown
  else spmm_lds<T, G, 0><<<nblocks, kLdsBlock, 0, stream>>>(b, nblocks, g_tuning.flags);
  SG_HIP_TRY(hipGetLastError());
  return SG_OK;
}

constexpr int kRingARow = 144;
constexpr int kRingAPiece = kLdsRows * kRingARow;

typedef __attribute__((ext_vector_type(8))) __bf16 ring_bf16x8;
typedef __attribute__((ext_vector_type(4))) __bf16 ring_bf16x4;
typedef __attribute__((ext_vector_type(4))) short ring_s16x4;

constexpr int kRingPieces = 3;
template <int ROWB, int NEPI, int D, int MODE>
struct RingLds {
  static constexpr int NP = kRingPieces;
  static constexpr int NREC = 2 * D;
  static constexpr int kSrc = kRingSlots * ROWB;
  static constexpr int kA = NP * kRingAPiece;
  static constexpr int kEpi = kLdsRows * ROWB;
  static constexpr int kStage = kSrc + kA + NEPI * kEpi;
  static constexpr int oA = kSrc;
  static constexpr int oEpi = kSrc + kA;
  static constexpr int oRec = D * kStage;
  static constexpr int oStg = oRec + NREC * kRecBytes;
  static constexpr int total = oStg + (MODE == 2 ? 2 : 0) * kLdsRows * ROWB;
  static_assert((64 - kRingSlots) * ROWB <= kA, "the rows the last MFMA step reads behind the source slots lie in the weight pieces");
};

__device__ __forceinline__ void ring_dma16(const void* src, uint8_t* lds) {
  __builtin_amdgcn_global_load_lds((const void __attribute__((address_space(1)))*)src,
                                   (void __attribute__((address_space(3)))*)lds, 16, 0, 0);
}
__device__ __forceinline__ int ring_swz(int row) { return (row & 3) | (((row >> 3) & 1) << 2); }
template <int N> __device__ __forceinline__ void ring_wait_vm() { asm volatile("s_waitcnt vmcnt(%0)" ::"n"(N) : "memory"); }
__device__ __forceinline__ void ring_wait_vm_n(int n) {
  switch (n) {
#define SG_RING_CASE(k) case k: ring_wait_vm<k>(); break;
    SG_RING_CASE(1) SG_RING_CASE(2) SG_RING_CASE(3) SG_RING_CASE(4) SG_RING_CASE(5) SG_RING_CASE(6) SG_RING_CASE(7) SG_RING_CASE(8)
    SG_RING_CASE(9) SG_RING_CASE(10) SG_RING_CASE(11) SG_RING_CASE(12) SG_RING_CASE(13) SG_RING_CASE(14) SG_RING_CASE(15) SG_RING_CASE(16)
    SG_RING_CASE(17) SG_RING_CASE(18) SG_RING_CASE(19) SG_RING_CASE(20) SG_RING_CASE(21) SG_RING_CASE(22) SG_RING_CASE(23) SG_RING_CASE(24)
    SG_RING_CASE(25) SG_RING_CASE(26) SG_RING_CASE(27) SG_RING_CASE(28) SG_RING_CASE(29) SG_RING_CASE(30) SG_RING_CASE(31) SG_RING_CASE(32)
#undef SG_RING_CASE
    default: ring_wait_vm<0>(); break;
  }
}
#define SG_RING_BARRIER()                                   \
  do {                                                      \
    asm volatile("s_waitcnt lgkmcnt(0)" ::: "memory");      \
    __builtin_amdgcn_s_barrier();                           \
    asm volatile("" ::: "memory");                          \
  } while (0)

template <int NBW, int NEPI, int D, int MODE>
__global__ __launch_bounds__(128 * NBW + 256) void spmm_ring(const SpmmArgs a, const int nt) {
  using V = Vt<bf16_tag>;
  constexpr int VEC = 8;
  constexpr int CW = 2 * NBW;
  constexpr int PW = 4;
  constexpr int C = 64 * NBW;
  constexpr int ROWB = 2 * C;
  constexpr int G = ROWB / 16;
  constexpr int RPW = 64 / G;
  constexpr int SRC_MAX = (kRingSlots / RPW + PW - 1) / PW;
  constexpr int EPI_PER_WAVE = kLdsRows / RPW / PW;
  constexpr int FIXED = NEPI * EPI_PER_WAVE + 1;
  static_assert(NBW == 2 || NBW == 4, "128 or 256 channels");
  static_assert(EPI_PER_WAVE * RPW * PW == kLdsRows && CW * RPW == kLdsRows, "equal shares");
  static_assert((D - 2) * (SRC_MAX + FIXED) <= 32 && D >= 2 && D <= 5, "vmcnt switch range");
  constexpr int NP = kRingPieces;
  static_assert(MODE == 0 || MODE == 2, "store modes");
  using L = RingLds<ROWB, NEPI, D, MODE>;
  using raw_t = typename V::raw;
  using elem_t = typename V::elem;

  __shared__ __attribute__((aligned(16))) uint8_t smem[L::total];

  const int tid = threadIdx.x, lane = tid & 63;
  const int wave = __builtin_amdgcn_readfirstlane(tid >> 6);

  const int xcd = blockIdx.x & 7, jb = blockIdx.x >> 3;
  const int nx = ((int)gridDim.x - xcd + 7) >> 3;
  const int q = nt >> 3, rem = nt & 7;
  const int tile_lo = xcd < rem ? xcd * (q + 1) : rem * (q + 1) + (xcd - rem) * q;
  const int tile_cnt = q + (xcd < rem ? 1 : 0);
  const int n_my = jb < tile_cnt ? (tile_cnt - jb + nx - 1) / nx : 0;
  if (n_my == 0) return;
  const int t_first = tile_lo + jb;

  const elem_t* __restrict__ X = (const elem_t*)a.X;

  for (int o = tid * 16; o < D * L::kStage; o += (CW + PW) * 64 * 16) *(u32x4*)(smem + o) = u32x4{0u, 0u, 0u, 0u};
  SG_RING_BARRIER();

  if (wave >= CW) {
    const int pw = wave - CW, ptid = tid - CW * 64;
    __builtin_amdgcn_s_setprio(3);
    const int g = lane / G, gl = lane % G;
    const elem_t* __restrict__ X0 = (const elem_t*)a.X0;
    const elem_t* __restrict__ X1 = (const elem_t*)a.X1;
    auto tile_of = [&](int k) { return t_first + (k < n_my ? k : n_my - 1) * nx; };
    auto issue_meta = [&](int tile, int slot) {
      constexpr int LPW = kRecBytes / 16 / PW;
      if (lane < LPW)
        ring_dma16(a.lt_rec + (int64_t)tile * kRecBytes + (pw * LPW + lane) * 16, smem + L::oRec + slot * kRecBytes + pw * LPW * 16);
    };
    int f_nu, f_src[SRC_MAX], f_erow[EPI_PER_WAVE];
    auto fetch = [&](int slot) {
      const uint8_t* rec = smem + L::oRec + slot * kRecBytes;
      f_nu = *(const int32_t*)(rec + kRecNu);
#pragma unroll
      for (int j = 0; j < SRC_MAX; ++j) {
        const int sl = (pw + PW * j) * RPW + g;
        f_src[j] = ((const int32_t*)(rec + kRecSrc))[sl < kRingSlots ? sl : kRingSlots - 1];
      }
#pragma unroll
      for (int j = 0; j < EPI_PER_WAVE; ++j) f_erow[j] = ((const int32_t*)(rec + kRecRow))[(pw + PW * j) * RPW + g];
    };
    uint32_t a_slots = 0xffffffffu;
    auto issue_tile = [&](int slot, int st) -> int {
      const uint8_t* rec = smem + L::oRec + slot * kRecBytes;
      uint8_t* stage = smem + st * L::kStage;
      const int nu = __builtin_amdgcn_readfirstlane(f_nu);
      const int n_inst = (nu + RPW - 1) / RPW;
      int issued = 0;
#pragma unroll
      for (int j = 0; j < SRC_MAX; ++j) {
        const int i = pw + PW * j;
        if (i < n_inst) {
          const int sl = i * RPW + g;
          const int chunk = ((((gl >> 1) ^ ring_swz(sl)) << 1) | (gl & 1));
          ring_dma16(X + (int64_t)f_src[j] * a.ldx + chunk * VEC, stage + i * (RPW * ROWB));
          ++issued;
        }
      }
      if (NEPI >= 1) {
#pragma unroll
        for (int j = 0; j < EPI_PER_WAVE; ++j) {
          const int i = pw + PW * j;
// ... 44 lines not shown
    }
    fetch(D - 1);
    asm volatile("" ::: "memory");
    int st = 0, rs = 0;
    for (int i = 0; i < n_my; ++i) {
      if (i == 0) {
        ring_wait_vm<0>();
      } else {
        int allowed = 0;
#pragma unroll
        for (int k = 0; k < D - 2; ++k) allowed += inflight[k];
        ring_wait_vm_n(allowed);
      }
      SG_RING_BARRIER();
      const int st_n = st == 0 ? D - 1 : st - 1;
      const int rs_n = rs + D - 1 >= L::NREC ? rs + D - 1 - L::NREC : rs + D - 1;
      const int rs_f = rs + D >= L::NREC ? rs + D - L::NREC : rs + D;
      const int rs_m = rs == 0 ? L::NREC - 1 : rs - 1;
      const int cnt = issue_tile(rs_n, st_n) + 1;
      issue_meta(tile_of(i + 2 * D - 1), rs_m);
      fetch(rs_f);
#pragma unroll
      for (int k = D - 2; k > 0; --k) inflight[k] = inflight[k - 1];
      inflight[0] = cnt;
      asm volatile("" ::: "memory");
      st = st + 1 == D ? 0 : st + 1;
      rs = rs + 1 == L::NREC ? 0 : rs + 1;
    }
    if (MODE == 2) SG_RING_BARRIER();
    ring_wait_vm<0>();
    return;
  }

  elem_t* __restrict__ Y = (elem_t*)a.Y;
  const uint32_t lds0 = (uint32_t)(uintptr_t)(const __attribute__((address_space(3))) uint8_t*)smem;
  const int m = lane & 15, fg = lane >> 4;
  const int fq = (lane >> 2) & 3, fp = lane & 3;
  const int col = wave * 32 + (fg & 1) * 16 + (fg >> 1) * 8;
  const int olr = wave * RPW + lane / G, ogl = lane % G;
  SG_RING_BARRIER();
  int c_nu, c_nrows, c_row, c_orow;
  float c_sd;
  auto fetch = [&](int slot) {
    const uint8_t* rec = smem + L::oRec + slot * kRecBytes;
    c_nu = *(const int32_t*)(rec + kRecNu);
    c_nrows = *(const int32_t*)(rec + kRecNrows);
    c_sd = ((const float*)(rec + kRecSd))[m];
    c_row = ((const int32_t*)(rec + kRecRow))[m];
    c_orow = ((const int32_t*)(rec + kRecRow))[olr];
  };
  fetch(0);
  int st = 0, rs = 0;
  int p_nrows = 0, p_orow = 0;
  for (int i = 0; i < n_my; ++i) {
    SG_RING_BARRIER();
    const uint8_t* rec = smem + L::oRec + rs * kRecBytes;
    uint8_t* stage = smem + st * L::kStage;
    const int nu = __builtin_amdgcn_readfirstlane(c_nu);
    const int nrows = __builtin_amdgcn_readfirstlane(c_nrows);
    const float sd = c_sd;
    const int row = c_row, orow = c_orow;
    raw_t out_prev = raw_t{0u, 0u, 0u, 0u};
    if (MODE == 2) out_prev = *(const raw_t*)(smem + L::oStg + ((i + 1) & 1) * (kLdsRows * ROWB) + olr * ROWB + ((ogl ^ (olr & 15)) << 4));
    const uint8_t* Ab = stage + L::oA;
    ring_bf16x8 wf0[NP];
    ring_s16x4 wf1[NP];
#pragma unroll
    for (int p = 0; p < NP; ++p) {
      wf0[p] = *(const ring_bf16x8*)(Ab + p * kRingAPiece + m * kRingARow + fg * 16);
      wf1[p] = *(const ring_s16x4*)(Ab + p * kRingAPiece + m * kRingARow + 64 + fg * 8);
    }
    raw_t x0v = raw_t{0u, 0u, 0u, 0u}, x1v = raw_t{0u, 0u, 0u, 0u};
    if (NEPI >= 1) x0v = *(const raw_t*)(stage + L::oEpi + m * ROWB + (((col >> 3) ^ m) << 4));
    if (NEPI >= 2) x1v = *(const raw_t*)(stage + L::oEpi + L::kEpi + m * ROWB + (((col >> 3) ^ m) << 4));
    fetch(rs + 1 == L::NREC ? 0 : rs + 1);
    const uint32_t xs = lds0 + st * L::kStage;
    ring_bf16x4 h0[2][2];
    ring_s16x4 h1[2];
    {
      const int sw = fq | ((fg & 1) << 2);
#pragma unroll
      for (int nb = 0; nb < 2; ++nb)
#pragma unroll
        for (int hh = 0; hh < 2; ++hh) {
          const uint32_t addr = xs + (uint32_t)((8 * fg + 4 * hh + fq) * ROWB + (((wave * 2 + nb) ^ sw) << 5) + fp * 8);
          asm volatile("ds_read_b64_tr_b16 %0, %1" : "=v"(h0[nb][hh]) : "v"(addr) : "memory");
        }
      const int sw1 = fq | (((fg >> 1) & 1) << 2);
#pragma unroll
      for (int nb = 0; nb < 2; ++nb) {
        const uint32_t addr = xs + (uint32_t)((32 + 4 * fg + fq) * ROWB + (((wave * 2 + nb) ^ sw1) << 5) + fp * 8);
        asm volatile("ds_read_b64_tr_b16 %0, %1" : "=v"(h1[nb]) : "v"(addr) : "memory");
      }
    }
    asm volatile("s_waitcnt lgkmcnt(0)" : "+v"(h0[0][0]), "+v"(h0[0][1]), "+v"(h0[1][0]), "+v"(h0[1][1]), "+v"(h1[0]), "+v"(h1[1])::"memory");
    if (MODE == 2) {
      if (olr < p_nrows) *(raw_t*)(Y + (int64_t)p_orow * a.ldy + ogl * VEC) = out_prev;
      p_nrows = nrows;
      p_orow = orow;
    }
    float v[8];
    if (nu > 0) {
      f32x4 acc[2] = {f32x4{0.f, 0.f, 0.f, 0.f}, f32x4{0.f, 0.f, 0.f, 0.f}};
#pragma unroll
      for (int p = 0; p < NP; ++p)
#pragma unroll
// ... 10 lines not shown
      if (nu > 48) {
        ring_s16x4 wf[NP];
#pragma unroll
        for (int p = 0; p < NP; ++p) wf[p] = *(const ring_s16x4*)(Ab + p * kRingAPiece + m * kRingARow + 96 + fg * 8);
        ring_s16x4 h[2];
        const int sw = fq | (((fg >> 1) & 1) << 2);
#pragma unroll
        for (int nb = 0; nb < 2; ++nb) {
          const uint32_t addr = xs + (uint32_t)((48 + 4 * fg + fq) * ROWB + (((wave * 2 + nb) ^ sw) << 5) + fp * 8);
          asm volatile("ds_read_b64_tr_b16 %0, %1" : "=v"(h[nb]) : "v"(addr) : "memory");
        }
        asm volatile("s_waitcnt lgkmcnt(0)" : "+v"(h[0]), "+v"(h[1])::"memory");
#pragma unroll
        for (int p = 0; p < NP; ++p)
#pragma unroll
          for (int nb = 0; nb < 2; ++nb) acc[nb] = __builtin_amdgcn_mfma_f32_16x16x16bf16_1k(h[nb], wf[p], acc[nb], 0, 0, 0);
      }
#pragma unroll
      for (int jj = 0; jj < 4; ++jj) {
        const auto r = __builtin_amdgcn_permlane16_swap(__float_as_uint(acc[0][jj]), __float_as_uint(acc[1][jj]), false, false);
        v[jj] = __uint_as_float(r[0]);
        v[4 + jj] = __uint_as_float(r[1]);
      }
    } else {
      const int r0 = *(const int32_t*)(rec + kRecR0);
#pragma unroll
      for (int c = 0; c < 8; ++c) v[c] = 0.f;
      if (m < nrows) {
        const int gs = a.rowptr[r0 + m], ge = a.rowptr[r0 + m + 1];
        for (int k = gs; k < ge; ++k) {
          const int2 e = a.lt_idx_w[k];
          float f[VEC];
          V::unpack(*(const raw_t*)(X + (int64_t)e.x * a.ldx + col), f);
          axpy<VEC>(__int_as_float(e.y), f, v);
        }
      }
    }
    const float sdst = a.alpha * sd;
    float y[VEC];
#pragma unroll
    for (int c = 0; c < VEC; ++c) y[c] = sdst * v[c];
    if (NEPI >= 1) {
      float f[VEC];
      V::unpack(x0v, f);
#pragma unroll
      for (int c = 0; c < VEC; ++c) y[c] = fmaf(a.beta, f[c], y[c]);
    }
    if (NEPI >= 2) {
      float f[VEC];
      V::unpack(x1v, f);
#pragma unroll
      for (int c = 0; c < VEC; ++c) y[c] = fmaf(a.gamma, f[c], y[c]);
    }
    if (MODE == 0) {
      if (m < nrows) *(raw_t*)(Y + (int64_t)row * a.ldy + col) = V::pack(y);
    } else {
      *(raw_t*)(smem + L::oStg + (i & 1) * (kLdsRows * ROWB) + m * ROWB + (((col >> 3) ^ m) << 4)) = V::pack(y);
    }
    st = st + 1 == D ? 0 : st + 1;
    rs = rs + 1 == L::NREC ? 0 : rs + 1;
  }
  if (MODE == 2) {
    SG_RING_BARRIER();
    const raw_t out = *(const raw_t*)(smem + L::oStg + ((n_my + 1) & 1) * (kLdsRows * ROWB) + olr * ROWB + ((ogl ^ (olr & 15)) << 4));
    if (olr < p_nrows) *(raw_t*)(Y + (int64_t)p_orow * a.ldy + ogl * VEC) = out;
  }
}

template <int NBW, int NEPI, int D, int MODE>
int launch_ring_k(const SpmmArgs& b, hipStream_t stream) {
  constexpr int lds = RingLds<128 * NBW, NEPI, D, MODE>::total;
  static_assert(lds <= 160 * 1024, "LDS budget");
  int per_cu = (160 * 1024) / lds;
  per_cu = per_cu > 4 ? 4 : per_cu;
  int64_t nb = (int64_t)per_cu * 256;
  if (nb > b.lt_nrec) nb = b.lt_nrec;
  nb = (nb + 7) / 8 * 8;
  spmm_ring<NBW, NEPI, D, MODE><<<(int)nb, 128 * NBW + 256, 0, stream>>>(b, b.lt_nrec);
  SG_HIP_TRY(hipGetLastError());
  return SG_OK;
}

template <int NBW>
int launch_ring(const SpmmArgs& a, hipStream_t stream) {
  SpmmArgs b = a;
  if (!a.X0 && a.X1) { b.X0 = a.X1; b.ldx0 = a.ldx1; b.beta = a.gamma; b.X1 = nullptr; b.ldx1 = 0; b.gamma = 0.f; }
  const int nepi = (b.X0 ? 1 : 0) + (b.X1 ? 1 : 0);
  const bool direct = (g_tuning.flags & kFlagRingDirectStores) != 0;
  if constexpr (NBW == 4) {
    if (nepi == 2) return launch_ring_k<NBW, 2, 3, 0>(b, stream);
    if (nepi == 1) return direct ? launch_ring_k<NBW, 1, 3, 0>(b, stream) : launch_ring_k<NBW, 1, 3, 2>(b, stream);
    return direct ? launch_ring_k<NBW, 0, 3, 0>(b, stream) : launch_ring_k<NBW, 0, 3, 2>(b, stream);
  } else {
    if (nepi == 2) return launch_ring_k<NBW, 2, 2, 0>(b, stream);
    if (nepi == 1) return launch_ring_k<NBW, 1, 3, 0>(b, stream);
    return direct ? launch_ring_k<NBW, 0, 3, 0>(b, stream) : launch_ring_k<NBW, 0, 3, 2>(b, stream);
  }
}

constexpr int kRingFARow = 272;
template <int ROWB, int NEPI, int D>
struct RingLdsF {
  static constexpr int NREC = 2 * D;
  static constexpr int kSrc = kRingSlots * ROWB;
  static constexpr int kA = kLdsRows * kRingFARow;
  static constexpr int kEpi = kLdsRows * ROWB;
  static constexpr int kStage = kSrc + kA + NEPI * kEpi;
  static constexpr int oA = kSrc;
  static constexpr int oEpi = kSrc + kA;
  static constexpr int oRec = D * kStage;
  static constexpr int total = oRec + NREC * kRecBytes;
};

template <int NBW, int NEPI, int D, int BPW>
__global__ __launch_bounds__(64 * (4 * NBW / BPW) + 256) void spmm_ring_f32(const SpmmArgs a, const int nt) {
  constexpr int CW = 4 * NBW / BPW;
  constexpr int PW = 4;
  constexpr int C = 64 * NBW;
  constexpr int ROWB = 4 * C;
  constexpr int G = ROWB / 16;
  constexpr int RPW = 64 / G;
  constexpr int SRC_MAX = (kRingSlots / RPW + PW - 1) / PW;
  constexpr int EPI_PER_WAVE = kLdsRows / RPW / PW;
  constexpr int FIXED = NEPI * EPI_PER_WAVE + 1;
  static_assert(NBW == 2 || NBW == 4, "128 or 256 channels");
  static_assert(EPI_PER_WAVE * RPW * PW == kLdsRows, "equal shares");
  static_assert((D - 2) * (SRC_MAX + FIXED) <= 32 && D >= 2 && D <= 5, "vmcnt switch range");
  using L = RingLdsF<ROWB, NEPI, D>;
  static_assert(L::total <= 160 * 1024, "LDS budget");

  __shared__ __attribute__((aligned(16))) uint8_t smem[L::total];
// ... 460 lines not shown
    while (ch > RPW && (int64_t)a.n_rows / ch < 4096) ch >>= 1;
  }
  if (ch < RPW) ch = RPW;
  if (ch > kChMax) ch = kChMax;
  ch = (ch / RPW) * RPW;
  const int64_t chunks = ((int64_t)a.n_rows + ch - 1) / ch;
  const int nblocks = (int)((chunks + kWaves - 1) / kWaves);
  constexpr int64_t esz = sizeof(typename Vt<T>::elem);
  const bool narrow = !(g_tuning.flags & kFlagWideAddr) && a.n_cols > 0 && a.n_cols < (1 << 24) &&
                      a.ldx * esz < (1 << 24) && a.n_cols * a.ldx * esz < ((int64_t)1 << 32);
  const int cap = g_tuning.unroll == 4 || g_tuning.unroll == 6 || g_tuning.unroll == 8 ? g_tuning.unroll : default_cap<T, G, R>();
#define SG_ROWS(NW, CP) spmm_rows<T, G, R, NEPI, NW, CP><<<nblocks, kBlock, 0, stream>>>(a, ch, nblocks, g_tuning.flags)
  if (!narrow) SG_ROWS(false, 8);
  else if (cap == 4) SG_ROWS(true, 4);
  else if (cap == 6) SG_ROWS(true, 6);
  else SG_ROWS(true, 8);
#undef SG_ROWS
  SG_HIP_TRY(hipGetLastError());
  return SG_OK;
}

template <typename T, int G, int R>
int launch_shared(const SpmmArgs& a, hipStream_t stream) {
  constexpr int MT = (64 / G) * kShTilesPerGroup;
  const int64_t n_mt = ((int64_t)a.n_rows + kTileRows - 1) / kTileRows;
  const int nblocks = (int)((n_mt + (int64_t)MT * kWaves - 1) / ((int64_t)MT * kWaves));
  SpmmArgs b = a;
  if (!a.X0 && a.X1) { b.X0 = a.X1; b.ldx0 = a.ldx1; b.beta = a.gamma; b.X1 = nullptr; b.ldx1 = 0; b.gamma = 0.f; }
  constexpr int64_t esz = sizeof(typename Vt<T>::elem);
  const bool narrow = !(g_tuning.flags & kFlagWideAddr) && a.n_cols > 0 && a.n_cols < (1 << 24) &&
                      a.ldx * esz < (1 << 24) && a.n_cols * a.ldx * esz < ((int64_t)1 << 32);
#define SG_SHARED(NE, NW) spmm_shared<T, G, R, NE, NW><<<nblocks, kBlock, 0, stream>>>(b, nblocks, g_tuning.flags)
  if (b.X0 && b.X1) { if (narrow) SG_SHARED(2, true); else SG_SHARED(2, false); }
  else if (b.X0) { if (narrow) SG_SHARED(1, true); else SG_SHARED(1, false); }
  else { if (narrow) SG_SHARED(0, true); else SG_SHARED(0, false); }
#undef SG_SHARED
  SG_HIP_TRY(hipGetLastError());
  return SG_OK;
}

template <typename T, int G, int R>
int launch_rows(const SpmmArgs& a, hipStream_t stream) {
  if (a.X0 && a.X1) return launch_rows_epi<T, G, R, 2>(a, stream);
  if (a.X0) return launch_rows_epi<T, G, R, 1>(a, stream);
  if (a.X1) {
    SpmmArgs b = a;
    b.X0 = a.X1; b.ldx0 = a.ldx1; b.beta = a.gamma; b.X1 = nullptr; b.ldx1 = 0; b.gamma = 0.f;
    return launch_rows_epi<T, G, R, 1>(b, stream);
  }
  return launch_rows_epi<T, G, R, 0>(a, stream);
}

template <typename T>
int launch_typed_one(const SpmmArgs& a, hipStream_t stream) {
  constexpr int VEC = Vt<T>::VEC;
  constexpr int esz = sizeof(typename Vt<T>::elem);
  const bool vec_ok = a.C % VEC == 0 && a.ldx % VEC == 0 && a.ldy % VEC == 0 && aligned16(a.X) &&
                      aligned16(a.Y) && (!a.X0 || (a.ldx0 % VEC == 0 && aligned16(a.X0))) &&
                      (!a.X1 || (a.ldx1 % VEC == 0 && aligned16(a.X1))) && a.C / VEC <= 256;
  (void)esz;
  if (esz == 2 && a.C == 4 && a.ldx % 4 == 0 && a.ldy % 4 == 0 && ((uintptr_t)a.X & 7) == 0 && ((uintptr_t)a.Y & 7) == 0 &&
      (!a.X0 || (a.ldx0 % 4 == 0 && ((uintptr_t)a.X0 & 7) == 0)) && (!a.X1 || (a.ldx1 % 4 == 0 && ((uintptr_t)a.X1 & 7) == 0)) &&
      !(g_tuning.flags & kFlagNoQuad)) {
    int nb = (a.n_rows + kBlock - 1) / kBlock;
    nb = nb > 256 * 64 ? 256 * 64 : nb;
    spmm_quad_bf16<<<nb, kBlock, 0, stream>>>(a);
    SG_HIP_TRY(hipGetLastError());
    return SG_OK;
  }
  if (!vec_ok) {
    const int64_t total = (int64_t)a.n_rows * a.C;
    int64_t nb = (total + kBlock - 1) / kBlock;
    if (nb > 256 * 32) nb = 256 * 32;
    spmm_scalar<T><<<(int)nb, kBlock, 0, stream>>>(a);
    SG_HIP_TRY(hipGetLastError());
    return SG_OK;
  }
  const int nvec = a.C / VEC;
  if (esz == 2 && (g_tuning.flags & kFlagThreadRows) && (nvec == 1 || nvec == 2 || nvec == 4)) {
    int nb = (a.n_rows + kBlock - 1) / kBlock;
    nb = nb > 256 * 64 ? 256 * 64 : nb;
    if (nvec == 1) spmm_thread_rows_bf16<1><<<nb, kBlock, 0, stream>>>(a);
    else if (nvec == 2) spmm_thread_rows_bf16<2><<<nb, kBlock, 0, stream>>>(a);
    else spmm_thread_rows_bf16<4><<<nb, kBlock, 0, stream>>>(a);
    SG_HIP_TRY(hipGetLastError());
    return SG_OK;
  }
  const int row_bytes = a.C * (int)sizeof(typename Vt<T>::elem);
  const int tmin = g_tuning.tiled_min_row_bytes;
  const bool forced = tmin < 0 && row_bytes >= -tmin;
  const bool pays = tmin > 0 && sizeof(typename Vt<T>::elem) == 4 && row_bytes >= tmin &&
                    (row_bytes >= 2 * tmin || !(a.X0 || a.X1));
  if (!(g_tuning.flags & kFlagNoRing) && esz == 2 && a.lt_rec && a.lt_nrec > 0 && a.n_cols < ((int64_t)1 << 31)) {
    if (a.C == 128) return launch_ring<2>(a, stream);
    if (a.C == 256) return launch_ring<4>(a, stream);
  }
  if (!(g_tuning.flags & (kFlagNoRing | kFlagNoRingF32)) && esz == 4 && a.lt_rec && a.lt_nrec > 0 && a.n_cols < ((int64_t)1 << 31)) {
    int rc = SG_OK;
    if ((a.C == 128 || a.C == 256) && launch_ring_f32(a, stream, &rc)) return rc;
  }
  if ((g_tuning.flags & kFlagLdsTiles) && a.lt_uptr && a.ldx % VEC == 0 && a.n_cols < ((int64_t)1 << 31)) {
    if (nvec == 16) return launch_lds<T, 16>(a, stream);
    if (nvec == 32) return launch_lds<T, 32>(a, stream);
    if (nvec == 64) return launch_lds<T, 64>(a, stream);
  }
  if (a.tile_uptr && (forced || pays) && !(g_tuning.flags & kFlagNoTiles)) {
    if (nvec > 16 && nvec <= 32) return launch_shared<T, 32, 1>(a, stream);
    if (nvec > 32 && nvec <= 64) return launch_shared<T, 64, 1>(a, stream);
    if (nvec > 64 && nvec <= 128) return launch_shared<T, 64, 2>(a, stream);
  }
  if (nvec <= 1) return launch_rows<T, 1, 1>(a, stream);
  if (nvec <= 2) return launch_rows<T, 2, 1>(a, stream);
  if (nvec <= 4) return launch_rows<T, 4, 1>(a, stream);
  if (nvec <= 8) return launch_rows<T, 8, 1>(a, stream);
  if (nvec <= 16) return launch_rows<T, 16, 1>(a, stream);
  if (nvec <= 32) return launch_rows<T, 32, 1>(a, stream);
  if (nvec <= 64) return launch_rows<T, 64, 1>(a, stream);
  if (nvec <= 128) return launch_rows<T, 64, 2>(a, stream);
  return launch_rows<T, 64, 4>(a, stream);
}

template <typename T>
int launch_typed(const SpmmArgs& a, hipStream_t stream) {
  constexpr int VEC = Vt<T>::VEC;
  const int slab = g_tuning.slab;
  if (slab <= 0 || a.C <= slab || slab % VEC != 0) return launch_typed_one<T>(a, stream);
  using elem_t = typename Vt<T>::elem;
  for (int c0 = 0; c0 < a.C; c0 += slab) {
    SpmmArgs s = a;
    s.C = a.C - c0 < slab ? a.C - c0 : slab;
    s.X = (const elem_t*)a.X + c0;
    s.Y = (elem_t*)a.Y + c0;
    if (a.X0) s.X0 = (const elem_t*)a.X0 + c0;
    if (a.X1) s.X1 = (const elem_t*)a.X1 + c0;
    int rc = launch_typed_one<T>(s, stream);
    if (rc != SG_OK) return rc;
  }
  return SG_OK;
}

}

bool tiles_enabled() { return g_tuning.tiled_min_row_bytes != 0; }
bool lds_tiles_enabled() { return (g_tuning.flags & kFlagLdsTiles) != 0; }
bool ring_enabled() { return (g_tuning.flags & kFlagNoRing) == 0; }
bool ring_f32_enabled() { return (g_tuning.flags & (kFlagNoRing | kFlagNoRingF32)) == 0; }

int set_tuning(int knob, int value) {
  switch (knob) {
    case SG_TUNE_CHUNK_ROWS: g_tuning.chunk_rows = value; return SG_OK;
    case SG_TUNE_FLAGS: g_tuning.flags = value; return SG_OK;
    case SG_TUNE_UNROLL: g_tuning.unroll = value; return SG_OK;
    case SG_TUNE_SLAB: g_tuning.slab = value; return SG_OK;
    case SG_TUNE_TILED_MIN_ROW_BYTES: g_tuning.tiled_min_row_bytes = value; return SG_OK;
    default: set_error("unknown tuning knob %d", knob); return SG_ERR_INVALID;
  }
}

int launch_spmm(const SpmmArgs& a_in, int dtype, hipStream_t stream) {
  if (a_in.n_rows == 0 || a_in.C == 0) return SG_OK;
  SpmmArgs a = a_in;
  if (g_tuning.flags & kFlagNoPackedScale) {
    a.idx_w = nullptr;
    a.tile_uniq_w = nullptr;
  }
  switch (dtype) {
    case SG_F32: return launch_typed<float>(a, stream);
    case SG_BF16: return launch_typed<bf16_tag>(a, stream);
    default: set_error("unsupported dtype %d", dtype); return SG_ERR_UNSUPPORTED;
  }
}

int launch_gather_rows(const int32_t* rows, int64_t n, const void* X, int64_t ldx, void* Y,
                       int64_t ldy, int64_t C, int dtype, hipStream_t stream) {
  if (n == 0 || C == 0) return SG_OK;
  auto run = [&](auto tag) -> int {
    using T = decltype(tag);
    constexpr int VEC = Vt<T>::VEC;
    const bool vec_ok = C % VEC == 0 && ldx % VEC == 0 && ldy % VEC == 0 && aligned16(X) && aligned16(Y);
    const int64_t total = vec_ok ? n * (C / VEC) : n * C;
    int64_t nb = (total + kBlock - 1) / kBlock;
    if (nb > 256 * 16) nb = 256 * 16;
    if (vec_ok)
      gather_rows_vec<T><<<(int)nb, kBlock, 0, stream>>>(rows, n, X, ldx, Y, ldy, (int)(C / VEC));
    else
      gather_rows_scalar<T><<<(int)nb, kBlock, 0, stream>>>(rows, n, X, ldx, Y, ldy, (int)C);
    SG_HIP_TRY(hipGetLastError());
    return SG_OK;
  };
  switch (dtype) {
    case SG_F32: return run(float{});
    case SG_BF16: return run(bf16_tag{});
    default: set_error("unsupported dtype %d", dtype); return SG_ERR_UNSUPPORTED;
  }
}

}
```

semigcn_amd/functional.py:

```python
from __future__ import annotations

import contextlib
import os
import weakref
from typing import Optional, Sequence

import torch

from . import capi
from .graph import MeshGraph


def _mm_f32_out(a: torch.Tensor, b: torch.Tensor) -> torch.Tensor:
    if a.dtype == torch.float32:
        return a @ b
    try:
        return torch.mm(a, b, out_dtype=torch.float32)
    except (TypeError, RuntimeError):
        return (a @ b).float()


def _bmm_f32_out(a: torch.Tensor, b: torch.Tensor) -> torch.Tensor:
    if a.dtype == torch.float32:
        return torch.bmm(a, b)
# ... 348 lines not shown
        ctx.graph, ctx.K, ctx.C = graph, K, C
        ctx.has_bias = bias is not None
        ctx.param_dtype = weights[0].dtype
        ctx.wcat_t = wcat_t
        ctx.params = (bias, *weights)
        ctx.save_for_backward(T, wcat)
        return out

    @staticmethod
    def backward(ctx, dout: torch.Tensor):
        T, wcat = ctx.saved_tensors
        graph, K, C = ctx.graph, ctx.K, ctx.C
        need_x, need_b = ctx.needs_input_grad[3], ctx.needs_input_grad[4]
        db = column_sums(dout).to(ctx.param_dtype) if (ctx.has_bias and need_b) else None
        dout = dout.contiguous()
        need_w = any(ctx.needs_input_grad[5:])
        dws = [None] * K
        if need_w:
            dwcat = weight_grad(dout, T).to(ctx.param_dtype)
            dws = [dwcat[:, k * C:(k + 1) * C] for k in range(K)]
        dx = None
        if need_x:
            dT = dense_nt(dout, ctx.wcat_t) if ctx.wcat_t is not None else dense_nn(dout, wcat)
            if K == 1:
                dx = dT
            else:
                g = [dT[:, k * C:(k + 1) * C] for k in range(K)]
                tr = not graph.symmetric
                for k in range(K - 2, 0, -1):
                    x1 = g[k + 2] if k + 2 <= K - 1 else None
                    graph.aggregate(g[k + 1], g[k], alpha=2.0, X0=g[k], beta=1.0, X1=x1, gamma=-1.0,
                                    transpose=tr)
                dx = torch.empty((T.shape[0], C), dtype=dout.dtype, device=dout.device)
                x1 = g[2] if K >= 3 else None
                graph.aggregate(g[1], dx, alpha=1.0, X0=g[0], beta=1.0, X1=x1, gamma=-1.0, transpose=tr)
        if dout.is_cuda and _sink(ctx.params, (db, *dws)):
            return (None, None, None, dx) + (None,) * (K + 1)
        return (None, None, None, dx, db, *dws)


def _wstack_set(weights, bias, dtype):
    K, Co = len(weights), weights[0].shape[0]
    ws = torch.cat(list(weights), dim=0).to(dtype)
    bk = None
    if bias is not None:
        bk = torch.cat([bias.float(), bias.new_zeros((K - 1) * Co, dtype=torch.float32)])
    wt = ws.t().contiguous() if dtype == torch.bfloat16 and ws.is_cuda and USE_MFMA_GEMM else None
    return ws, bk, wt


class _ChebConvPostFn(torch.autograd.Function):

    @staticmethod
    def forward(ctx, graph: MeshGraph, cache: Optional[WeightCache], x, bias, *weights):
        K = len(weights)
        Co = weights[0].shape[0]

        def build():
            return _wstack_set(weights, bias, x.dtype)
        wstack, bias_k, wstack_t = build() if cache is None else cache.get("stack", x.dtype, weights, bias, build)
        x = x if x.stride(1) == 1 else x.contiguous()
        Z = dense_nt(x, wstack, bias_k)
        z = [Z[:, k * Co:(k + 1) * Co] for k in range(K)]
        for k in range(K - 2, 0, -1):
            x1 = z[k + 2] if k + 2 <= K - 1 else None
            graph.aggregate(z[k + 1], z[k], alpha=2.0, X0=z[k], beta=1.0, X1=x1, gamma=-1.0)
        out = torch.empty((x.shape[0], Co), dtype=x.dtype, device=x.device)
        graph.aggregate(z[1], out, alpha=1.0, X0=z[0], beta=1.0, X1=z[2] if K >= 3 else None, gamma=-1.0)
        ctx.graph, ctx.K, ctx.Co = graph, K, Co
        ctx.has_bias, ctx.param_dtype = bias is not None, weights[0].dtype
        ctx.wstack_t = wstack_t
        ctx.params = (bias, *weights)
        ctx.save_for_backward(x, wstack)
        return out

    @staticmethod
    def backward(ctx, dout):
        x, wstack = ctx.saved_tensors
        graph, K, Co = ctx.graph, ctx.K, ctx.Co
        V = dout.shape[0]
        tr = not graph.symmetric
        db = column_sums(dout).to(ctx.param_dtype) if (ctx.has_bias and ctx.needs_input_grad[3]) else None
        G = _adopt_wide(dout, K)
        if G is None:
            dout = dout.contiguous()
            G = torch.empty((V, K * Co), dtype=dout.dtype, device=dout.device)
            G[:, :Co].copy_(dout)
        g = [G[:, k * Co:(k + 1) * Co] for k in range(K)]
        dout = g[0]
        graph.aggregate(g[0], g[1], alpha=1.0, transpose=tr)
        for k in range(2, K):
            graph.aggregate(g[k - 1], g[k], alpha=2.0, X0=g[k - 2], beta=-1.0, transpose=tr)
        dx = None
        if ctx.needs_input_grad[2]:
            dx = dense_nt(G, ctx.wstack_t) if ctx.wstack_t is not None else dense_nn(G, wstack)
        dws = [None] * K
        if any(ctx.needs_input_grad[4:]):
            dwstack = weight_grad(G, x.contiguous()).to(ctx.param_dtype)
            dws = [dwstack[k * Co:(k + 1) * Co] for k in range(K)]
        if dout.is_cuda and _sink(ctx.params, (db, *dws)):
            return (None, None, dx) + (None,) * (K + 1)
        return (None, None, dx, db, *dws)


AGGREGATE_AFTER_GEMM_WHEN_NARROWING = True


def cheb_conv(graph: MeshGraph, x: torch.Tensor, weights: Sequence[torch.Tensor],
              bias: Optional[torch.Tensor] = None, cache: Optional[WeightCache] = None,
              moments: Optional[dict] = None) -> torch.Tensor:
    if x.dim() != 2:
        raise ValueError(f"x must be [V, C], got {tuple(x.shape)}")
    if getattr(graph, "sg_partitioned", False):
        from .dist import dist_cheb_conv
        return dist_cheb_conv(graph, x, weights, bias, cache, moments)
    if x.shape[0] != graph.num_vertices:
        raise ValueError(f"x has {x.shape[0]} rows but the graph has {graph.num_vertices} vertices")
    if AGGREGATE_AFTER_GEMM_WHEN_NARROWING and len(weights) >= 2 and weights[0].shape[0] < weights[0].shape[1]:
        return _ChebConvPostFn.apply(graph, cache, x, bias, *weights)
    return _ChebConvFn.apply(graph, cache, moments, x, bias, *weights)


class _LaplacianFn(torch.autograd.Function):

    @staticmethod
    def forward(ctx, graph: MeshGraph, x, alpha: float, x0, beta: float):
        x = x.contiguous() if x.stride(-1) != 1 else x
        y = torch.empty((graph.handle.num_rows, x.shape[1]), dtype=x.dtype, device=x.device)
        graph.aggregate(x, y, alpha=alpha, X0=x0, beta=beta)
        ctx.graph, ctx.alpha, ctx.beta = graph, alpha, beta
        return y

    @staticmethod
    def backward(ctx, dy):
        g = ctx.graph
        dy = dy.contiguous()
        dx = None
        if ctx.needs_input_grad[1]:
            dx = torch.empty((g.handle.num_cols, dy.shape[1]), dtype=dy.dtype, device=dy.device)
            g.aggregate(dy, dx, alpha=ctx.alpha, transpose=not g.symmetric)
        dx0 = ctx.beta * dy if ctx.needs_input_grad[3] else None
        return None, dx, None, dx0, None


def laplacian_apply(graph: MeshGraph, x, alpha: float = 1.0, x0=None, beta: float = 0.0):
    return _LaplacianFn.apply(graph, x, alpha, x0, beta)


class _PoolFn(torch.autograd.Function):
    @staticmethod
    def forward(ctx, pool: capi.PoolHandle, x, mode: str):
        ctx.pool, ctx.mode = pool, mode
        return pool.pool_mean(x) if mode == "pool" else pool.unpool(x)

    @staticmethod
    def backward(ctx, dy):
        dy = dy.contiguous()
        dx = ctx.pool.pool_mean_bwd(dy) if ctx.mode == "pool" else ctx.pool.unpool_bwd(dy)
        return None, dx, None


def mesh_pool(pool: capi.PoolHandle, x: torch.Tensor) -> torch.Tensor:
    return _PoolFn.apply(pool, x, "pool")


def mesh_unpool(pool: capi.PoolHandle, x: torch.Tensor) -> torch.Tensor:
    return _PoolFn.apply(pool, x, "unpool")


class _BNActFn(torch.autograd.Function):
    @staticmethod
    def forward(ctx, x, weight, bias, running_mean, running_var, training, momentum, eps, slope, group, widen,
                grad_widen=1, rows=0, tile_moments=None, batches_tracked=None):
        V, C = x.shape
        if x.stride(1) != 1 and C > 1:
            x = x.contiguous()
        dev = x.device
        w32 = weight if weight.dtype == torch.float32 else weight.float()
        b32 = bias if bias.dtype == torch.float32 else bias.float()
        if training and V > 1 and not ctx_group_active(group):
            if tile_moments is not None:
                fin = capi.bn_stats_finalize_tiles(tile_moments["tiles"], tile_moments["rows"], V, w32, b32, running_mean,
                                                   running_var, momentum, eps, batches_tracked)
            else:
                fin = capi.bn_stats_finalize(capi.col_moments(x), V, w32, b32, running_mean, running_var, momentum, eps,
                                             batches_tracked)
            mean, invstd, scale, shift = fin[0], fin[1], fin[2], fin[3]
            ctx.N = float(V)
        elif training and ctx_group_active(group):
            from . import dist as _d
            import torch.distributed as tdist
            world = tdist.get_world_size(group)
            local = torch.empty((1, 2 * C + 1), dtype=torch.float32, device=dev)
            if tile_moments is not None:
                capi.bn_local_stats(tile_moments["tiles"], tile_moments["rows"], V, local)
            else:
                capi.bn_local_stats(capi.col_moments(x), 0, V, local)
            allst = torch.empty((world, 2 * C + 1), dtype=torch.float32, device=dev)
            _d._all_gather_rows(allst, local, group)
            fin, n_dev = capi.bn_finalize_ranks(allst, w32, b32, running_mean, running_var, momentum, eps, batches_tracked)
            mean, invstd, scale, shift = fin[0], fin[1], fin[2], fin[3]
            ctx.N = n_dev
        elif training:
            if batches_tracked is not None:
                batches_tracked.add_(1)
            stats = capi.bn_merge(capi.col_moments(x), V)
            fin = capi.bn_finalize(stats, float(V), w32, b32, running_mean, running_var, momentum, eps)
            mean, invstd, scale, shift = fin[0], fin[1], fin[2], fin[3]
            ctx.N = float(V)
        else:
            mean = running_mean.float()
            invstd = torch.rsqrt(running_var.float() + eps)
            scale = (w32 * invstd).contiguous()
            shift = (b32 - mean * scale).contiguous()
            ctx.N = float(V)
        if widen > 1:
            y = _new_wide(max(rows, V), V, C, widen, x.dtype, dev)
        else:
            y = torch.empty((V, C), dtype=x.dtype, device=dev)
        capi.scale_shift_act(x, scale, shift, slope, out=y)
        for obs in bn_act_observers:
            obs(y)
        ctx.save_for_backward(x, scale, shift, mean, invstd, w32)
        ctx.training, ctx.slope, ctx.group, ctx.param_dtype = training, slope, group, weight.dtype
        ctx.grad_widen = grad_widen
        ctx.params = (weight, bias)
        return y

    @staticmethod
    def backward(ctx, dy):
        x, scale, shift, mean, invstd, w32 = ctx.saved_tensors
        if dy.stride(1) != 1 and dy.shape[1] > 1:
            dy = dy.contiguous()
        part = capi.bn_act_bwd_reduce(dy, x, scale, shift, mean, invstd, ctx.slope)
        nothing = (None,) * 12
        if ctx.training and not ctx_group_active(ctx.group):
            weight, bias = ctx.params
            sunk = bool(_sink_depth) and ctx.needs_input_grad[1] and ctx.needs_input_grad[2] and all(
                p.grad is not None and p.grad.dtype == torch.float32 and p.grad.is_contiguous() and p.grad.device == x.device
                for p in (weight, bias))
            co = capi.bn_bwd_coeffs(part, ctx.N, w32, invstd, weight.grad if sunk else None, bias.grad if sunk else None)
            out = None
            if ctx.grad_widen > 1:
                out = _new_wide(x.shape[0], x.shape[0], x.shape[1], ctx.grad_widen, x.dtype, x.device)
            if FUSE_BIAS_GRAD:
                dx, sums = capi.bn_act_bwd_apply_colsum(dy, x, scale, shift, mean, invstd, co[4], co[2], co[3], ctx.slope,
                                                        out=out)
# ... 738 lines not shown
```

semigcn_amd/nn.py:

```python
from __future__ import annotations

import math
from typing import List, Optional, Sequence, Tuple, Union

import torch
import torch.nn as nn
from torch import Tensor

from . import functional as F_sg
from .graph import MeshGraph, graph_for


class _GlorotLinear(nn.Module):

    def __init__(self, in_channels: int, out_channels: int):
        super().__init__()
        self.in_channels, self.out_channels = in_channels, out_channels
        self.weight = nn.Parameter(torch.empty(out_channels, in_channels))
        self.reset_parameters()

    def reset_parameters(self):
        bound = math.sqrt(6.0 / (self.in_channels + self.out_channels))
        nn.init.uniform_(self.weight, -bound, bound)

# ... 202 lines not shown
        i, n = _start, len(self._plan)
        blocks_on = F_sg.blocks_enabled()
        while i < n:
            name, ins, outs = self._plan[i]
            vals = [scope[a] for a in ins]
            on_dev = len(vals) >= 1 and torch.is_tensor(vals[0]) and vals[0].is_cuda and vals[0].dim() == 2
            if on_dev and len(vals) == 2 and blocks_on and getattr(vals[1], "phases", False) and self.training:
                plans, j = [], i
                while j < n and self._plan[j][1] == ins and self._plan[j][2] == outs:
                    nxt = self._block_at(j)
                    if nxt is None or nxt[0].pool is not None:
                        break
                    plans.append(nxt[0])
                    j = nxt[1] + 1
                if plans:
                    from .dist import part_blocks
                    y = part_blocks(plans, vals[1], vals[0])
                    if y is not None:
                        scope[outs[0]] = result = y
                        i = j
                        continue
            if on_dev and len(vals) == 2 and blocks_on:
                blk = self._block_at(i)
                if blk is not None and blk[0].usable(vals[0]):
                    g = vals[1]
                    if not isinstance(g, MeshGraph):
                        g = None if getattr(g, "sg_partitioned", False) or not torch.is_tensor(g) else graph_for(g, vals[0].shape[0])
                    if g is not None:
                        plans, last = [blk[0]], blk
                        while F_sg.chaining_allowed():
                            j = last[1] + 1
                            nxt = self._block_at(j) if (j < n and self._plan[j][1] == ins and self._plan[j][2] == outs) else None
                            if nxt is None or last[0].pool is not None \
                                    or not nxt[0].usable_for(vals[0].dtype, vals[0].device, vals[0].shape[0], last[0].Cout):
                                break
                            plans.append(nxt[0])
                            last = nxt
                        scope[outs[0]] = result = F_sg.cheb_chain(plans, [g] * len(plans), vals[0], last[2])
                        i = last[1] + 1
                        continue
            fused = self._fusable_at(i) if (len(vals) == 1 and on_dev) else None
            mod = getattr(self, name)
            if fused is not None:
                part = next((v for v in scope.values() if getattr(v, "sg_partitioned", False)), None)
                tiles = pending[1] if (pending is not None and pending[0] is vals[0]) else None
                result = F_sg.bn_act(vals[0], mod, fused[0], fused[1],
                                     1 if part is not None else fused[2], 0 if part is None else part.n_ext,
                                     tile_moments=tiles)
                i += 1
            elif isinstance(mod, ChebConv) and on_dev and mod.training and self._fusable_at(i + 1) is not None \
                    and self._plan[i + 1][1] == outs:
                mom = {}
                result = mod(*vals, moments=mom)
                pending = (result, mom) if "tiles" in mom else None
            else:
                result = mod(*vals)
            if len(outs) == 1:
                scope[outs[0]] = result
            else:
                scope.update(zip(outs, result))
            i += 1
        return result

    def __len__(self):
        return len(self._plan)

    def __getitem__(self, i: int):
        return getattr(self, self._plan[i][0])


def _as_graph(g, rows: int):
    if not isinstance(g, MeshGraph):
        if getattr(g, "sg_partitioned", False) or not torch.is_tensor(g):
            return None
        g = graph_for(g, rows)
    return g if g.num_vertices == rows else None


def run_sequentials(pairs, x):
    if torch.is_tensor(x) and x.is_cuda and x.dim() == 2 and len(pairs) > 1 and F_sg.blocks_enabled() and F_sg.chaining_allowed() \
            and x.shape[0] <= F_sg.CHAIN_MAX_ROWS:
        plans, graphs, rows, cin, end, widen = [], [], x.shape[0], x.shape[1], None, 1
        for k, (seq, g) in enumerate(pairs):
            lead = seq._leading_blocks() if isinstance(seq, Sequential) else None
            gg = _as_graph(g, rows) if lead is not None else None
            if gg is None:
                break
            r, c = rows, cin
            for p in lead[0]:
                if not p.usable_for(x.dtype, x.device, r, c):
                    r = -1
                    break
                r, c = p.rows_out(r), p.Cout
            if r < 0:
                break
            plans.extend(lead[0])
            graphs.extend([gg] * len(lead[0]))
            rows, cin, end, widen = r, c, (k, lead[1]), lead[2]
            if lead[1] < len(seq):
                break
        if end is not None and len(plans) > 1:
            x = F_sg.cheb_chain(plans, graphs, x, widen)
            seq, g = pairs[end[0]]
            if end[1] < len(seq):
                x = seq(x, g, _start=end[1])
            pairs = pairs[end[0] + 1:]
    for seq, g in pairs:
# ... 3 lines not shown
```

Baseline: 38.12 iter/s.

## Fuse BatchNorm column moments into final ring SpMM epilogue

```diff
diff --git a/include/semigcn.h b/include/semigcn.h
--- a/include/semigcn.h
+++ b/include/semigcn.h
@@ -60,6 +60,14 @@
 SG_API int sg_spmm(const sg_graph* g, int transpose, const void* X, int64_t ldx, const void* X0,
             int64_t ldx0, const void* X1, int64_t ldx1, void* Y, int64_t ldy, int64_t C, int dtype,
             float alpha, float beta, float gamma, void* stream);
+SG_API int64_t sg_spmm_moment_records(const sg_graph* g, int64_t C, int dtype);
+SG_API int sg_spmm_moments(const sg_graph* g, int transpose, const void* X, int64_t ldx, const void* X0, int64_t ldx0,
+                           const void* X1, int64_t ldx1, void* Y, int64_t ldy, int64_t C, int dtype, float alpha,
+                           float beta, float gamma, float* moments, int* moments_done, void* stream);
+SG_API int sg_bn_stats_finalize_counted(const float* records, int64_t n_records, int64_t V, int64_t C, const float* gamma,
+                                        const float* beta, float* running_mean, float* running_var, float momentum, float eps,
+                                        float* out, int64_t* batches_tracked, void* stream);
+SG_API int64_t sg_col_moment_launches(void);
 
 SG_API int sg_pool_create(const int64_t* fine, const int64_t* coarse, int64_t n, int64_t n_fine,
                    int64_t n_coarse, void* stream, sg_pool** out);
diff --git a/semigcn_amd/capi.py b/semigcn_amd/capi.py
--- a/semigcn_amd/capi.py
+++ b/semigcn_amd/capi.py
@@ -77,6 +77,12 @@
     "sg_graph_export": (c_int, [c_void_p, c_void_p, c_void_p, c_void_p, c_void_p]),
     "sg_spmm": (c_int, [c_void_p, c_int, c_void_p, c_int64, c_void_p, c_int64, c_void_p, c_int64,
                         c_void_p, c_int64, c_int64, c_int, c_float, c_float, c_float, c_void_p]),
+    "sg_spmm_moment_records": (c_int64, [c_void_p, c_int64, c_int]),
+    "sg_spmm_moments": (c_int, [c_void_p, c_int, c_void_p, c_int64, c_void_p, c_int64, c_void_p, c_int64,
+                                c_void_p, c_int64, c_int64, c_int, c_float, c_float, c_float, c_void_p, POINTER(c_int), c_void_p]),
+    "sg_bn_stats_finalize_counted": (c_int, [c_void_p, c_int64, c_int64, c_int64, c_void_p, c_void_p, c_void_p, c_void_p,
+                                             c_float, c_float, c_void_p, c_void_p, c_void_p]),
+    "sg_col_moment_launches": (c_int64, []),
     "sg_graph_prepare": (c_int, [c_void_p, c_int64, c_int, c_void_p]),
     "sg_pool_create": (c_int, [c_void_p, c_void_p, c_int64, c_int64, c_int64, c_void_p, POINTER(c_void_p)]),
     "sg_pool_destroy": (c_int, [c_void_p]),
@@ -386,7 +392,9 @@
 
     def spmm(self, X: torch.Tensor, Y: torch.Tensor, *, alpha: float = 1.0, X0: Optional[torch.Tensor] = None,
              beta: float = 0.0, X1: Optional[torch.Tensor] = None, gamma: float = 0.0,
-             transpose: bool = False) -> torch.Tensor:
+             transpose: bool = False, moments: Optional[dict] = None) -> torch.Tensor:
+        if moments is not None:
+            return self._spmm_moments(X, Y, alpha, X0, beta, X1, gamma, transpose, moments)
         if _timer is None and X.is_cuda and X.dim() == 2 and Y.dim() == 2 and X.device.index == _current_device():
             dt = X.dtype
             code = _DTYPES.get(dt)
@@ -414,6 +422,38 @@
                     _check(rc, "sg_spmm")
                 return Y
         return self._spmm_checked(X, Y, alpha, X0, beta, X1, gamma, transpose)
+
+    def moment_records(self, C: int, dtype: torch.dtype) -> int:
+        code = _DTYPES.get(dtype)
+        return 0 if code is None else int(load().sg_spmm_moment_records(self._h, int(C), code))
+
+    def _spmm_moments(self, X, Y, alpha, X0, beta, X1, gamma, transpose, moments: dict) -> torch.Tensor:
+        R = self.moment_records(X.shape[1], X.dtype) if (X.is_cuda and X.dim() == 2) else 0
+        if R == 0:
+            return self.spmm(X, Y, alpha=alpha, X0=X0, beta=beta, X1=X1, gamma=gamma, transpose=transpose)
+        for t, n in ((X, "X"), (Y, "Y"), (X0, "X0"), (X1, "X1")):
+            if t is not None:
+                _require_device(t, n)
+                if t.dtype != X.dtype:
+                    raise SemigcnLibraryError(f"{n} dtype {t.dtype} != X dtype {X.dtype}")
+        C = X.shape[1]
+        n_in, n_out = (self.num_rows, self.num_cols) if transpose else (self.num_cols, self.num_rows)
+        if X.shape[0] != n_in or Y.shape != (n_out, C):
+            raise SemigcnLibraryError(f"spmm shape mismatch: X {tuple(X.shape)} Y {tuple(Y.shape)} operator {n_out}x{n_in}")
+        for t, n in ((X0, "X0"), (X1, "X1")):
+            if t is not None and t.shape != (n_out, C):
+                raise SemigcnLibraryError(f"{n} shape {tuple(t.shape)} != {(n_out, C)}")
+        rec = torch.empty((R * (3 * C + 1),), dtype=torch.float32, device=X.device)
+        done = c_int(0)
+        with _on_device(X.device):
+            _check(load().sg_spmm_moments(self._h, int(transpose), _ptr(X), _rows2d(X, "X"),
+                                          _ptr(X0), 0 if X0 is None else _rows2d(X0, "X0"),
+                                          _ptr(X1), 0 if X1 is None else _rows2d(X1, "X1"),
+                                          _ptr(Y), _rows2d(Y, "Y"), C, dtype_code(X), float(alpha), float(beta), float(gamma),
+                                          _ptr(rec), ctypes.byref(done), _stream(X)), "sg_spmm_moments")
+        if done.value:
+            moments["records"] = rec
+        return Y
 
     def _spmm_checked(self, X, Y, alpha, X0, beta, X1, gamma, transpose) -> torch.Tensor:
         for t, n in ((X, "X"), (Y, "Y"), (X0, "X0"), (X1, "X1")):
@@ -647,6 +687,29 @@
                                            float(momentum), float(eps), _ptr(out), _counter(batches_tracked, partial),
                                            _stream(partial)), "sg_bn_stats_finalize")
     return out
+
+
+def bn_stats_finalize_counted(records: torch.Tensor, num_rows: int, gamma: torch.Tensor, beta: torch.Tensor,
+                              running_mean: Optional[torch.Tensor], running_var: Optional[torch.Tensor], momentum: float,
+                              eps: float, batches_tracked: Optional[torch.Tensor] = None) -> torch.Tensor:
+    C = gamma.numel()
+    R = records.numel() // (3 * C + 1)
+    if records.dtype != torch.float32 or not records.is_contiguous() or R < 1 or R * (3 * C + 1) != records.numel():
+        raise SemigcnLibraryError("bn_stats_finalize_counted: records must be R * (3C + 1) contiguous floats")
+    out = torch.empty((4, C), dtype=torch.float32, device=records.device)
+    for t, n in ((running_mean, "running_mean"), (running_var, "running_var")):
+        if t is not None:
+            _f32vec(t, C, n)
+    with _on_device(records.device):
+        _check(load().sg_bn_stats_finalize_counted(_ptr(records), R, int(num_rows), C, _ptr(_f32vec(gamma, C, "weight")),
+                                                   _ptr(_f32vec(beta, C, "bias")), _ptr(running_mean), _ptr(running_var),
+                                                   float(momentum), float(eps), _ptr(out), _counter(batches_tracked, records),
+                                                   _stream(records)), "sg_bn_stats_finalize_counted")
+    return out
+
+
+def col_moment_launches() -> int:
+    return int(load().sg_col_moment_launches())
 
 
 def bn_stats_finalize_tiles(partial: torch.Tensor, rows_per_tile: int, num_rows: int, gamma: torch.Tensor,
diff --git a/semigcn_amd/csrc/api.hip b/semigcn_amd/csrc/api.hip
--- a/semigcn_amd/csrc/api.hip
+++ b/semigcn_amd/csrc/api.hip
@@ -68,7 +68,7 @@
 int run_csr(const Csr& c, const float* sd, const float* ss, const void* X, int64_t ldx,
             const void* X0, int64_t ldx0, const void* X1, int64_t ldx1, void* Y, int64_t ldy,
             int64_t C, int dtype, float alpha, float beta, float gamma, hipStream_t stream,
-            const int32_t* row_id = nullptr) {
+            const int32_t* row_id = nullptr, float* moments = nullptr, bool* moments_done = nullptr) {
   SG_REQUIRE(C >= 0 && C <= INT32_MAX, "C out of range");
   if (c.n_rows == 0 || C == 0) return SG_OK;
   int rc;
@@ -112,7 +112,8 @@
   a.n_cols = c.n_cols;
   a.C = (int32_t)C;
   a.alpha = alpha; a.beta = beta; a.gamma = gamma;
-  return launch_spmm(a, dtype, stream);
+  a.moments = moments;
+  return launch_spmm(a, dtype, stream, moments_done);
 }
 
 }
@@ -332,10 +333,21 @@
   return SG_OK;
 }
 
-SG_API int sg_spmm(const sg_graph* g, int transpose, const void* X, int64_t ldx, const void* X0, int64_t ldx0,
-            const void* X1, int64_t ldx1, void* Y, int64_t ldy, int64_t C, int dtype, float alpha,
-            float beta, float gamma, void* stream) {
+SG_API int64_t sg_spmm_moment_records(const sg_graph* g, int64_t C, int dtype) {
+  return (g && g->square && ring_moment_floats(C, dtype) > 0) ? kRingMomentRecords : 0;
+}
+
+SG_API int sg_spmm_moments(const sg_graph* g, int transpose, const void* X, int64_t ldx, const void* X0, int64_t ldx0,
+                           const void* X1, int64_t ldx1, void* Y, int64_t ldy, int64_t C, int dtype, float alpha,
+                           float beta, float gamma, float* moments, int* moments_done, void* stream) {
   SG_REQUIRE(g != nullptr, "sg_spmm: null graph");
+  bool done_b = false;
+  if (!(moments && moments_done && g->square && ring_moment_floats(C, dtype) > 0)) moments = nullptr;
+  bool* const done = moments ? &done_b : nullptr;
+  struct Report {
+    int* out; const bool* v;
+    ~Report() { if (out) *out = *v ? 1 : 0; }
+  } report{moments_done, &done_b};
   const bool t = transpose != 0;
   if (t && !g->square) {
     set_error("sg_spmm: transpose of a rectangular (partition) operator is not available; "
@@ -346,13 +358,19 @@
                    (hipStream_t)stream);
   if (g->square && g->symmetric && g->row_id && g->loc.rowptr)
     return run_csr(g->loc, g->dis_dst_loc, g->dis_src, X, ldx, X0, ldx0, X1, ldx1, Y, ldy, C, dtype, -alpha, beta, gamma,
-                   (hipStream_t)stream, g->row_id);
+                   (hipStream_t)stream, g->row_id, moments, done);
   if (!g->square && g->row_id)
     return run_csr(g->fwd, g->dis_dst, g->dis_src, X, ldx, X0, ldx0, X1, ldx1, Y, ldy, C, dtype, -alpha, beta, gamma,
                    (hipStream_t)stream, g->row_id);
   const Csr& c = (t && !g->symmetric) ? g->bwd : g->fwd;
   return run_csr(c, g->dis_dst, g->dis_src, X, ldx, X0, ldx0, X1, ldx1, Y, ldy, C, dtype, -alpha,
-                 beta, gamma, (hipStream_t)stream);
+                 beta, gamma, (hipStream_t)stream, nullptr, moments, done);
+}
+
+SG_API int sg_spmm(const sg_graph* g, int transpose, const void* X, int64_t ldx, const void* X0, int64_t ldx0,
+            const void* X1, int64_t ldx1, void* Y, int64_t ldy, int64_t C, int dtype, float alpha,
+            float beta, float gamma, void* stream) {
+  return sg_spmm_moments(g, transpose, X, ldx, X0, ldx0, X1, ldx1, Y, ldy, C, dtype, alpha, beta, gamma, nullptr, nullptr, stream);
 }
 
 SG_API int sg_graph_prepare(const sg_graph* g, int64_t C, int dtype, void* stream) {
@@ -568,6 +586,18 @@
   return launch_bn_stats_finalize(partial, nb, V, C, gamma, beta, running_mean, running_var, momentum, eps, out,
                                   batches_tracked, (hipStream_t)stream);
 }
+
+SG_API int sg_bn_stats_finalize_counted(const float* records, int64_t n_records, int64_t V, int64_t C, const float* gamma,
+                                        const float* beta, float* running_mean, float* running_var, float momentum, float eps,
+                                        float* out, int64_t* batches_tracked, void* stream) {
+  SG_REQUIRE(V > 1 && C >= 0 && n_records > 0 && records && gamma && beta && out, "sg_bn_stats_finalize_counted: bad argument");
+  SG_REQUIRE((running_mean == nullptr) == (running_var == nullptr),
+             "sg_bn_stats_finalize_counted: give both running buffers or none");
+  return launch_bn_stats_finalize_counted(records, n_records, V, C, gamma, beta, running_mean, running_var, momentum, eps, out,
+                                          batches_tracked, (hipStream_t)stream);
+}
+
+SG_API int64_t sg_col_moment_launches(void) { return col_moment_launches(); }
 
 SG_API int sg_bn_stats_finalize_tiles(const float* partial, int64_t n_tiles, int64_t rows_per_tile, int64_t V, int64_t C,
                                       const float* gamma, const float* beta, float* running_mean, float* running_var,
diff --git a/semigcn_amd/csrc/block.hip b/semigcn_amd/csrc/block.hip
--- a/semigcn_amd/csrc/block.hip
+++ b/semigcn_amd/csrc/block.hip
@@ -164,6 +164,8 @@
   const int64_t R = gemm_tile_rows(s->Co);
   const int64_t tiles = (s->V + R - 1) / R;
   s->mom_floats = (tiles > s->nb ? tiles : s->nb) * 2 * s->Co;
+  const int64_t ring = b.order == 1 ? sg_spmm_moment_records(b.graph, s->Co, b.dtype) * (3 * s->Co + 1) : 0;
+  if (ring > s->mom_floats) s->mom_floats = ring;
   return SG_OK;
 }
 
@@ -270,6 +272,7 @@
 
   void* const Hc = b.pool_mode ? w.Hc : b.H;
   bool tile_moments = false;
+  int ring_moments = 0;
   if (b.order == 0) {
     Planes pt;
     if ((rc = t_layout(b, s, "sg_block_forward", &pt)) != SG_OK) return rc;
@@ -296,7 +299,9 @@
                 stream);
       if (rc != SG_OK) return rc;
     }
-    rc = spmm(b, false, z(1), ldz, z(0), ldz, b.K >= 3 ? z(2) : nullptr, ldz, Hc, s.Co, s.Co, 1.f, 1.f, -1.f, stream);
+    const bool want = b.training && b.pool_mode == 0;
+    rc = sg_spmm_moments(b.graph, 0, z(1), ldz, z(0), ldz, b.K >= 3 ? z(2) : nullptr, ldz, Hc, s.Co, s.Co, b.dtype, 1.f, 1.f, -1.f,
+                         want ? w.moments : nullptr, want ? &ring_moments : nullptr, (void*)stream);
     if (rc != SG_OK) return rc;
   }
   if (b.pool_mode == 1) rc = sg_pool_mean(b.pool, Hc, s.Co, b.H, s.Co, s.Co, b.dtype, (void*)stream);
@@ -308,6 +313,9 @@
       const int64_t R = gemm_tile_rows(s.Co);
       rc = launch_bn_stats_finalize_tiles(w.moments, (s.V + R - 1) / R, R, s.Vo, s.Co, b.gamma, b.beta, b.running_mean,
                                           b.running_var, b.momentum, b.eps, b.stats, b.batches_tracked, stream);
+    } else if (ring_moments) {
+      rc = launch_bn_stats_finalize_counted(w.moments, sg_spmm_moment_records(b.graph, s.Co, b.dtype), s.Vo, s.Co, b.gamma, b.beta,
+                                            b.running_mean, b.running_var, b.momentum, b.eps, b.stats, b.batches_tracked, stream);
     } else {
       rc = launch_col_reduce(0, b.H, s.Co, nullptr, 0, nullptr, nullptr, nullptr, nullptr, 0.f, w.moments, s.nb, s.Vo, s.Co,
                              b.dtype, stream);
diff --git a/semigcn_amd/csrc/bn_act.hip b/semigcn_amd/csrc/bn_act.hip
--- a/semigcn_amd/csrc/bn_act.hip
+++ b/semigcn_amd/csrc/bn_act.hip
@@ -398,16 +398,25 @@
                                                          const float* __restrict__ beta, float* running_mean,
                                                          float* running_var, float momentum, float eps,
                                                          float* __restrict__ out ,
-                                                         long long* batches_tracked) {
+                                                         long long* batches_tracked,
+                                                         const float* __restrict__ counts = nullptr) {
   __shared__ double s_n[4], s_mean[4], s_m2[4];
   const int lane = threadIdx.x & 63, wave = threadIdx.x >> 6;
   const int c = blockIdx.x;
   double n = 0.0, mean = 0.0, m2 = 0.0;
   for (int64_t b = threadIdx.x; b < nb; b += 256) {
-    int64_t rows = V - b * rpb;
-    rows = rows > rpb ? rpb : rows;
-    if (rows <= 0) break;
-    const double nbk = (double)rows, mb = partial[(b * 2 + 0) * C + c], qb = partial[(b * 2 + 1) * C + c];
+    int64_t rows;
+    if (counts) {
+      rows = (int64_t)counts[b];
+      if (rows <= 0) continue;
+    } else {
+      rows = V - b * rpb;
+      rows = rows > rpb ? rpb : rows;
+      if (rows <= 0) break;
+    }
+    const double nbk = (double)rows;
+    const double mb = counts ? (double)partial[(b * 3 + 0) * C + c] + (double)partial[(b * 3 + 1) * C + c] : (double)partial[(b * 2 + 0) * C + c];
+    const double qb = counts ? partial[(b * 3 + 2) * C + c] : partial[(b * 2 + 1) * C + c];
     const double tot = n + nbk, delta = mb - mean;
     mean += delta * (nbk / tot);
     m2 += qb + delta * delta * (n * nbk / tot);
@@ -594,6 +603,17 @@
   return SG_OK;
 }
 
+int launch_bn_stats_finalize_counted(const float* partial, int64_t nb, int64_t V, int64_t C, const float* gamma,
+                                     const float* beta, float* running_mean, float* running_var, float momentum, float eps,
+                                     float* out, int64_t* batches_tracked, hipStream_t stream) {
+  if (C == 0) return SG_OK;
+  SG_REQUIRE(nb > 0, "counted moments need at least one record");
+  bn_stats_finalize<<<(int)C, 256, 0, stream>>>(partial, nb, V, (int)C, 0, gamma, beta, running_mean, running_var, momentum,
+                                                eps, out, (long long*)batches_tracked, partial + nb * 3 * C);
+  SG_HIP_TRY(hipGetLastError());
+  return SG_OK;
+}
+
 int launch_multi_add(int n, const float* const* srcs, const int64_t* src_ld, const int64_t* rows, const int64_t* cols,
                      float* const* dsts, hipStream_t stream) {
   MultiAddArgs a{};
@@ -647,10 +667,14 @@
   return SG_OK;
 }
 
+static std::atomic<int64_t> g_col_moment_launches{0};
+int64_t col_moment_launches() { return g_col_moment_launches.load(std::memory_order_relaxed); }
+
 int launch_col_reduce(int mode, const void* A, int64_t lda, const void* H, int64_t ldh, const float* scale,
                       const float* shift, const float* mean, const float* invstd, float slope, float* out,
                       int64_t nblk, int64_t V, int64_t C, int dtype, hipStream_t stream) {
   if (V == 0 || C == 0) return SG_OK;
+  if (mode == 0) g_col_moment_launches.fetch_add(1, std::memory_order_relaxed);
   SG_REQUIRE(nblk == col_blocks(V), "partial buffer must have sg_col_blocks(V) = %lld blocks", (long long)col_blocks(V));
   const int rpb = (int)((V + nblk - 1) / nblk);
   auto run = [&](auto dt_tag) -> int {
diff --git a/semigcn_amd/csrc/sg_common.h b/semigcn_amd/csrc/sg_common.h
--- a/semigcn_amd/csrc/sg_common.h
+++ b/semigcn_amd/csrc/sg_common.h
@@ -79,6 +79,7 @@
 constexpr int kRecSd = kRecNrows + 4;
 constexpr int kRecRow = kRecSd + 4 * kLdsRows;
 constexpr int kRecW = kRecRow + 4 * kLdsRows;
+constexpr int kRingMomentRecords = 1024;
 constexpr int kRecBytes = 896;
 static_assert(kRecW + 4 * kRingSlots <= kRecBytes && kRecSd % 16 == 0, "tile record layout");
 int build_tiles(Csr* c, hipStream_t stream);
@@ -172,9 +173,11 @@
   int64_t n_cols = 0;
   int32_t C;
   float alpha, beta, gamma;
-};
-
-int launch_spmm(const SpmmArgs& a, int dtype, hipStream_t stream);
+  float* moments = nullptr;
+};
+
+int launch_spmm(const SpmmArgs& a, int dtype, hipStream_t stream, bool* moments_done = nullptr);
+int64_t ring_moment_floats(int64_t C, int dtype);
 int set_tuning(int knob, int value);
 bool tiles_enabled();
 bool lds_tiles_enabled();
@@ -189,6 +192,10 @@
 int launch_bn_stats_finalize(const float* partial, int64_t nb, int64_t V, int64_t C, const float* gamma,
                              const float* beta, float* running_mean, float* running_var, float momentum, float eps,
                              float* out, int64_t* batches_tracked, hipStream_t stream);
+int launch_bn_stats_finalize_counted(const float* partial, int64_t nb, int64_t V, int64_t C, const float* gamma,
+                                     const float* beta, float* running_mean, float* running_var, float momentum, float eps,
+                                     float* out, int64_t* batches_tracked, hipStream_t stream);
+int64_t col_moment_launches();
 int launch_bn_bwd_coeffs(const float* partial, int64_t nb, int64_t C, double N, const float* gamma,
                          const float* invstd, float* out, float* acc_dweight, float* acc_dbias, const float* count_dev,
                          hipStream_t stream);
diff --git a/semigcn_amd/csrc/spmm.hip b/semigcn_amd/csrc/spmm.hip
--- a/semigcn_amd/csrc/spmm.hip
+++ b/semigcn_amd/csrc/spmm.hip
@@ -711,7 +711,7 @@
     asm volatile("" ::: "memory");                          \
   } while (0)
 
-template <int NBW, int NEPI, int D, int MODE>
+template <int NBW, int NEPI, int D, int MODE, bool MOM>
 __global__ __launch_bounds__(128 * NBW + 256) void spmm_ring(const SpmmArgs a, const int nt) {
   using V = Vt<bf16_tag>;
   constexpr int VEC = 8;
@@ -744,6 +744,10 @@
   const int tile_lo = xcd < rem ? xcd * (q + 1) : rem * (q + 1) + (xcd - rem) * q;
   const int tile_cnt = q + (xcd < rem ? 1 : 0);
   const int n_my = jb < tile_cnt ? (tile_cnt - jb + nx - 1) / nx : 0;
+  if (MOM && threadIdx.x == 0) {
+    float* cnt = a.moments + (int64_t)kRingMomentRecords * 3 * C;
+    for (int s = blockIdx.x + (n_my == 0 ? 0 : (int)gridDim.x); s < kRingMomentRecords; s += (int)gridDim.x) cnt[s] = 0.f;
+  }
   if (n_my == 0) return;
   const int t_first = tile_lo + jb;
 
@@ -894,6 +898,9 @@
   fetch(0);
   int st = 0, rs = 0;
   int p_nrows = 0, p_orow = 0;
+  float mo_n = 0.f, mo_k[VEC], mo_mean[VEC], mo_m2[VEC];
+#pragma unroll
+  for (int c = 0; c < VEC; ++c) { mo_k[c] = 0.f; mo_mean[c] = 0.f; mo_m2[c] = 0.f; }
   for (int i = 0; i < n_my; ++i) {
     SG_RING_BARRIER();
     const uint8_t* rec = smem + L::oRec + rs * kRecBytes;
@@ -1010,10 +1017,30 @@
 #pragma unroll
       for (int c = 0; c < VEC; ++c) y[c] = fmaf(a.gamma, f[c], y[c]);
     }
+    const raw_t yp = V::pack(y);
     if (MODE == 0) {
-      if (m < nrows) *(raw_t*)(Y + (int64_t)row * a.ldy + col) = V::pack(y);
+      if (m < nrows) *(raw_t*)(Y + (int64_t)row * a.ldy + col) = yp;
     } else {
-      *(raw_t*)(smem + L::oStg + (i & 1) * (kLdsRows * ROWB) + m * ROWB + (((col >> 3) ^ m) << 4)) = V::pack(y);
+      *(raw_t*)(smem + L::oStg + (i & 1) * (kLdsRows * ROWB) + m * ROWB + (((col >> 3) ^ m) << 4)) = yp;
+    }
+    if (MOM) {
+      float xr[VEC];
+      V::unpack(yp, xr);
+      if (i == 0) {
+#pragma unroll
+        for (int c = 0; c < VEC; ++c) mo_k[c] = __shfl(xr[c], 0, 16);
+      }
+      if (m < nrows) {
+        mo_n += 1.f;
+        const float rn = __builtin_amdgcn_rcpf(mo_n);
+#pragma unroll
+        for (int c = 0; c < VEC; ++c) {
+          const float x = xr[c] - mo_k[c];
+          const float d = x - mo_mean[c];
+          mo_mean[c] = fmaf(d, rn, mo_mean[c]);
+          mo_m2[c] = fmaf(d, x - mo_mean[c], mo_m2[c]);
+        }
+      }
     }
     st = st + 1 == D ? 0 : st + 1;
     rs = rs + 1 == L::NREC ? 0 : rs + 1;
@@ -1022,6 +1049,33 @@
     SG_RING_BARRIER();
     const raw_t out = *(const raw_t*)(smem + L::oStg + ((n_my + 1) & 1) * (kLdsRows * ROWB) + olr * ROWB + ((ogl ^ (olr & 15)) << 4));
     if (olr < p_nrows) *(raw_t*)(Y + (int64_t)p_orow * a.ldy + ogl * VEC) = out;
+  }
+  if (MOM) {
+#pragma unroll
+    for (int off = 8; off > 0; off >>= 1) {
+      const float n2 = __shfl_down(mo_n, off, 16);
+      const float tot = mo_n + n2;
+      const float f2 = tot > 0.f ? n2 / tot : 0.f;
+      const float fx = mo_n * f2;
+#pragma unroll
+      for (int c = 0; c < VEC; ++c) {
+        const float mean2 = __shfl_down(mo_mean[c], off, 16), m22 = __shfl_down(mo_m2[c], off, 16);
+        const float d = mean2 - mo_mean[c];
+        mo_mean[c] = fmaf(d, f2, mo_mean[c]);
+        mo_m2[c] = (mo_m2[c] + m22) + d * d * fx;
+      }
+      mo_n = tot;
+    }
+    if (m == 0) {
+      float* recm = a.moments + (int64_t)blockIdx.x * 3 * C;
+      *(f32x4*)(recm + col) = f32x4{mo_k[0], mo_k[1], mo_k[2], mo_k[3]};
+      *(f32x4*)(recm + col + 4) = f32x4{mo_k[4], mo_k[5], mo_k[6], mo_k[7]};
+      *(f32x4*)(recm + C + col) = f32x4{mo_mean[0], mo_mean[1], mo_mean[2], mo_mean[3]};
+      *(f32x4*)(recm + C + col + 4) = f32x4{mo_mean[4], mo_mean[5], mo_mean[6], mo_mean[7]};
+      *(f32x4*)(recm + 2 * C + col) = f32x4{mo_m2[0], mo_m2[1], mo_m2[2], mo_m2[3]};
+      *(f32x4*)(recm + 2 * C + col + 4) = f32x4{mo_m2[4], mo_m2[5], mo_m2[6], mo_m2[7]};
+      if (tid == 0) a.moments[(int64_t)kRingMomentRecords * 3 * C + blockIdx.x] = mo_n;
+    }
   }
 }
 
@@ -1032,9 +1086,11 @@
   int per_cu = (160 * 1024) / lds;
   per_cu = per_cu > 4 ? 4 : per_cu;
   int64_t nb = (int64_t)per_cu * 256;
+  static_assert(4 * 256 <= kRingMomentRecords, "one moments record per workgroup");
   if (nb > b.lt_nrec) nb = b.lt_nrec;
   nb = (nb + 7) / 8 * 8;
-  spmm_ring<NBW, NEPI, D, MODE><<<(int)nb, 128 * NBW + 256, 0, stream>>>(b, b.lt_nrec);
+  if (b.moments) spmm_ring<NBW, NEPI, D, MODE, true><<<(int)nb, 128 * NBW + 256, 0, stream>>>(b, b.lt_nrec);
+  else spmm_ring<NBW, NEPI, D, MODE, false><<<(int)nb, 128 * NBW + 256, 0, stream>>>(b, b.lt_nrec);
   SG_HIP_TRY(hipGetLastError());
   return SG_OK;
 }
@@ -1601,7 +1657,10 @@
 }
 
 template <typename T>
-int launch_typed_one(const SpmmArgs& a, hipStream_t stream) {
+int launch_typed_one(const SpmmArgs& a_in, hipStream_t stream, bool* moments_done) {
+  SpmmArgs a = a_in;
+  float* const moments = a_in.moments;
+  a.moments = nullptr;
   constexpr int VEC = Vt<T>::VEC;
   constexpr int esz = sizeof(typename Vt<T>::elem);
   const bool vec_ok = a.C % VEC == 0 && a.ldx % VEC == 0 && a.ldy % VEC == 0 && aligned16(a.X) &&
@@ -1641,8 +1700,11 @@
   const bool pays = tmin > 0 && sizeof(typename Vt<T>::elem) == 4 && row_bytes >= tmin &&
                     (row_bytes >= 2 * tmin || !(a.X0 || a.X1));
   if (!(g_tuning.flags & kFlagNoRing) && esz == 2 && a.lt_rec && a.lt_nrec > 0 && a.n_cols < ((int64_t)1 << 31)) {
-    if (a.C == 128) return launch_ring<2>(a, stream);
-    if (a.C == 256) return launch_ring<4>(a, stream);
+    if (a.C == 128 || a.C == 256) {
+      a.moments = moments_done ? moments : nullptr;
+      if (a.moments) *moments_done = true;
+      return a.C == 128 ? launch_ring<2>(a, stream) : launch_ring<4>(a, stream);
+    }
   }
   if (!(g_tuning.flags & (kFlagNoRing | kFlagNoRingF32)) && esz == 4 && a.lt_rec && a.lt_nrec > 0 && a.n_cols < ((int64_t)1 << 31)) {
     int rc = SG_OK;
@@ -1670,10 +1732,10 @@
 }
 
 template <typename T>
-int launch_typed(const SpmmArgs& a, hipStream_t stream) {
+int launch_typed(const SpmmArgs& a, hipStream_t stream, bool* moments_done) {
   constexpr int VEC = Vt<T>::VEC;
   const int slab = g_tuning.slab;
-  if (slab <= 0 || a.C <= slab || slab % VEC != 0) return launch_typed_one<T>(a, stream);
+  if (slab <= 0 || a.C <= slab || slab % VEC != 0) return launch_typed_one<T>(a, stream, moments_done);
   using elem_t = typename Vt<T>::elem;
   for (int c0 = 0; c0 < a.C; c0 += slab) {
     SpmmArgs s = a;
@@ -1682,7 +1744,7 @@
     s.Y = (elem_t*)a.Y + c0;
     if (a.X0) s.X0 = (const elem_t*)a.X0 + c0;
     if (a.X1) s.X1 = (const elem_t*)a.X1 + c0;
-    int rc = launch_typed_one<T>(s, stream);
+    int rc = launch_typed_one<T>(s, stream, nullptr);
     if (rc != SG_OK) return rc;
   }
   return SG_OK;
@@ -1706,7 +1768,12 @@
   }
 }
 
-int launch_spmm(const SpmmArgs& a_in, int dtype, hipStream_t stream) {
+int64_t ring_moment_floats(int64_t C, int dtype) {
+  return (dtype == SG_BF16 && (C == 128 || C == 256)) ? (int64_t)kRingMomentRecords * (3 * C + 1) : 0;
+}
+
+int launch_spmm(const SpmmArgs& a_in, int dtype, hipStream_t stream, bool* moments_done) {
+  if (moments_done) *moments_done = false;
   if (a_in.n_rows == 0 || a_in.C == 0) return SG_OK;
   SpmmArgs a = a_in;
   if (g_tuning.flags & kFlagNoPackedScale) {
@@ -1714,8 +1781,8 @@
     a.tile_uniq_w = nullptr;
   }
   switch (dtype) {
-    case SG_F32: return launch_typed<float>(a, stream);
-    case SG_BF16: return launch_typed<bf16_tag>(a, stream);
+    case SG_F32: return launch_typed<float>(a, stream, nullptr);
+    case SG_BF16: return launch_typed<bf16_tag>(a, stream, moments_done);
     default: set_error("unsupported dtype %d", dtype); return SG_ERR_UNSUPPORTED;
   }
 }
diff --git a/semigcn_amd/functional.py b/semigcn_amd/functional.py
--- a/semigcn_amd/functional.py
+++ b/semigcn_amd/functional.py
@@ -424,7 +424,7 @@
 class _ChebConvPostFn(torch.autograd.Function):
 
     @staticmethod
-    def forward(ctx, graph: MeshGraph, cache: Optional[WeightCache], x, bias, *weights):
+    def forward(ctx, graph: MeshGraph, cache: Optional[WeightCache], moments: Optional[dict], x, bias, *weights):
         K = len(weights)
         Co = weights[0].shape[0]
 
@@ -438,7 +438,10 @@
             x1 = z[k + 2] if k + 2 <= K - 1 else None
             graph.aggregate(z[k + 1], z[k], alpha=2.0, X0=z[k], beta=1.0, X1=x1, gamma=-1.0)
         out = torch.empty((x.shape[0], Co), dtype=x.dtype, device=x.device)
-        graph.aggregate(z[1], out, alpha=1.0, X0=z[0], beta=1.0, X1=z[2] if K >= 3 else None, gamma=-1.0)
+        if moments is not None and isinstance(graph, MeshGraph):
+            graph.aggregate(z[1], out, alpha=1.0, X0=z[0], beta=1.0, X1=z[2] if K >= 3 else None, gamma=-1.0, moments=moments)
+        else:
+            graph.aggregate(z[1], out, alpha=1.0, X0=z[0], beta=1.0, X1=z[2] if K >= 3 else None, gamma=-1.0)
         ctx.graph, ctx.K, ctx.Co = graph, K, Co
         ctx.has_bias, ctx.param_dtype = bias is not None, weights[0].dtype
         ctx.wstack_t = wstack_t
@@ -452,7 +455,7 @@
         graph, K, Co = ctx.graph, ctx.K, ctx.Co
         V = dout.shape[0]
         tr = not graph.symmetric
-        db = column_sums(dout).to(ctx.param_dtype) if (ctx.has_bias and ctx.needs_input_grad[3]) else None
+        db = column_sums(dout).to(ctx.param_dtype) if (ctx.has_bias and ctx.needs_input_grad[4]) else None
         G = _adopt_wide(dout, K)
         if G is None:
             dout = dout.contiguous()
@@ -464,15 +467,15 @@
         for k in range(2, K):
             graph.aggregate(g[k - 1], g[k], alpha=2.0, X0=g[k - 2], beta=-1.0, transpose=tr)
         dx = None
-        if ctx.needs_input_grad[2]:
+        if ctx.needs_input_grad[3]:
             dx = dense_nt(G, ctx.wstack_t) if ctx.wstack_t is not None else dense_nn(G, wstack)
         dws = [None] * K
-        if any(ctx.needs_input_grad[4:]):
+        if any(ctx.needs_input_grad[5:]):
             dwstack = weight_grad(G, x.contiguous()).to(ctx.param_dtype)
             dws = [dwstack[k * Co:(k + 1) * Co] for k in range(K)]
         if dout.is_cuda and _sink(ctx.params, (db, *dws)):
-            return (None, None, dx) + (None,) * (K + 1)
-        return (None, None, dx, db, *dws)
+            return (None, None, None, dx) + (None,) * (K + 1)
+        return (None, None, None, dx, db, *dws)
 
 
 AGGREGATE_AFTER_GEMM_WHEN_NARROWING = True
@@ -489,7 +492,7 @@
     if x.shape[0] != graph.num_vertices:
         raise ValueError(f"x has {x.shape[0]} rows but the graph has {graph.num_vertices} vertices")
     if AGGREGATE_AFTER_GEMM_WHEN_NARROWING and len(weights) >= 2 and weights[0].shape[0] < weights[0].shape[1]:
-        return _ChebConvPostFn.apply(graph, cache, x, bias, *weights)
+        return _ChebConvPostFn.apply(graph, cache, moments, x, bias, *weights)
     return _ChebConvFn.apply(graph, cache, moments, x, bias, *weights)
 
 
@@ -551,7 +554,10 @@
         w32 = weight if weight.dtype == torch.float32 else weight.float()
         b32 = bias if bias.dtype == torch.float32 else bias.float()
         if training and V > 1 and not ctx_group_active(group):
-            if tile_moments is not None:
+            if tile_moments is not None and "records" in tile_moments:
+                fin = capi.bn_stats_finalize_counted(tile_moments["records"], V, w32, b32, running_mean, running_var,
+                                                     momentum, eps, batches_tracked)
+            elif tile_moments is not None:
                 fin = capi.bn_stats_finalize_tiles(tile_moments["tiles"], tile_moments["rows"], V, w32, b32, running_mean,
                                                    running_var, momentum, eps, batches_tracked)
             else:
@@ -564,7 +570,7 @@
             import torch.distributed as tdist
             world = tdist.get_world_size(group)
             local = torch.empty((1, 2 * C + 1), dtype=torch.float32, device=dev)
-            if tile_moments is not None:
+            if tile_moments is not None and "tiles" in tile_moments:
                 capi.bn_local_stats(tile_moments["tiles"], tile_moments["rows"], V, local)
             else:
                 capi.bn_local_stats(capi.col_moments(x), 0, V, local)
diff --git a/semigcn_amd/nn.py b/semigcn_amd/nn.py
--- a/semigcn_amd/nn.py
+++ b/semigcn_amd/nn.py
@@ -278,7 +278,7 @@
                     and self._plan[i + 1][1] == outs:
                 mom = {}
                 result = mod(*vals, moments=mom)
-                pending = (result, mom) if "tiles" in mom else None
+                pending = (result, mom) if ("tiles" in mom or "records" in mom) else None
             else:
                 result = mod(*vals)
             if len(outs) == 1:
```

Measured after the change: 38.25 iter/s (median of 6 runs). No clear change (+0.3%).
